# DataIntensive-HPC/abft-sparse-cg

Hardware: AMD Instinct MI355X
Metric: CG iterations/sec + SpMV effective HBM GB/s (% of roofline), 1/2/4/8 MI355X (higher is better)
Workload: dtype f64; 1 GPU; cg-csr -t hip -m none, synthetic laplace5:3162,3162; N=9998244, nnz=49978572, format=csr, mode=none, parallelism=1 GPU

## Files before the change

abft_sparse_cg_amd/capi.py:

```python
import ctypes as C
import os

_HERE = os.path.dirname(os.path.abspath(__file__))
LIB_PATH = os.environ.get("ABFT_HIP_LIB") or os.path.join(_HERE, "libabft_hip.so")
HEADER_PATH = os.path.join(os.path.dirname(_HERE), "include", "abft_hip.h")

OK = 0
MODES = ("none", "constraints", "sed", "sec7", "sec8", "secded")
MODE_ID = {m: i for i, m in enumerate(MODES)}
MODE_ID["sec"] = MODE_ID["sec7"]
FMT_CSR, FMT_COO = 0, 1
FLIP_ANY, FLIP_VALUE, FLIP_INDEX = 0, 1, 2
PART_ALL, PART_INTERIOR, PART_BOUNDARY = 0, 1, 2
K_SPMV, K_DOT, K_CALC_XR, K_CALC_P = 0, 1, 2, 3
EV_VEC_CORRECTED, EV_VEC_DOUBLE = 10, 11
FMT_VECTOR = 2
MAX_RHS = 8

u32p = C.POINTER(C.c_uint32)
f64p = C.POINTER(C.c_double)
i32p = C.POINTER(C.c_int)
vp = C.c_void_p
vpp = C.POINTER(C.c_void_p)

# ... 9 lines not shown

    def tup(self):
        return (self.kind, self.index, self.bit)


SIGNATURES = {
    "abft_hip_last_error": (C.c_char_p, []),
    "abft_hip_device_count": (C.c_int, [i32p]),
    "abft_hip_init": (C.c_int, [C.c_int, vpp]),
    "abft_hip_shutdown": (C.c_int, [vp]),
    "abft_hip_set_stream": (C.c_int, [vp, vp]),
    "abft_hip_get_stream": (vp, [vp]),
    "abft_hip_synchronize": (C.c_int, [vp]),
    "abft_hip_synchronize_timeout": (C.c_int, [vp, C.c_double]),
    "abft_hip_matrix_create_csr": (C.c_int, [vp, C.c_int, u32p, u32p, f64p, C.c_int, C.c_int, vpp]),
    "abft_hip_matrix_create_coo": (C.c_int, [vp, C.c_int, u32p, u32p, f64p, C.c_int, C.c_int, vpp]),
    "abft_hip_matrix_create_shard": (C.c_int, [vp, C.c_int, C.c_int, u32p, u32p, f64p, C.c_int, C.c_int,
                                               C.c_int, C.c_uint32, vpp]),
    "abft_hip_matrix_create_shard_indexed": (C.c_int, [vp, C.c_int, C.c_int, u32p, u32p, f64p, C.c_int, C.c_int,
                                                       C.c_int, u32p, vpp]),
    "abft_hip_matrix_destroy": (C.c_int, [vp]),
    "abft_hip_matrix_info": (C.c_int, [vp, i32p, i32p]),
    "abft_hip_matrix_compact_stats": (C.c_int, [vp, u32p, u32p, u32p]),
    "abft_hip_matrix_packed_stats": (C.c_int, [vp, u32p, u32p, u32p]),
    "abft_hip_matrix_read_element": (C.c_int, [vp, C.c_uint32, u32p]),
    "abft_hip_matrix_read_csr": (C.c_int, [vp, vp, vp, vp]),
    "abft_hip_matrix_read_coo": (C.c_int, [vp, vp]),
    "abft_hip_inject": (C.c_int, [vp, C.c_uint32, i32p, C.c_int]),
    "abft_hip_inject_rowptr": (C.c_int, [vp, C.c_uint32, C.c_uint32]),
    "abft_hip_vector_create": (C.c_int, [vp, C.c_int, vpp]),
    "abft_hip_vector_view": (C.c_int, [vp, C.c_int, C.c_int, vpp]),
    "abft_hip_vector_destroy": (C.c_int, [vp]),
    "abft_hip_vector_map": (C.c_int, [vp, C.POINTER(f64p)]),
    "abft_hip_vector_unmap": (C.c_int, [vp, f64p]),
    "abft_hip_vector_copy": (C.c_int, [vp, vp]),
    "abft_hip_vector_device_ptr": (vp, [vp]),
    "abft_hip_vector_length": (C.c_int, [vp]),
    "abft_hip_dot": (C.c_int, [vp, vp, vp, f64p]),
    "abft_hip_calc_xr": (C.c_int, [vp, vp, vp, vp, vp, C.c_double, f64p]),
    "abft_hip_calc_p": (C.c_int, [vp, vp, vp, C.c_double]),
    "abft_hip_spmv": (C.c_int, [vp, vp, vp, vp]),
    "abft_hip_matrix_create_csr_stream": (C.c_int, [vp, C.c_int, u32p, u32p, f64p, C.c_int, C.c_int, vpp]),
    "abft_hip_spmm": (C.c_int, [vp, vp, vp, vp, C.c_int]),
    "abft_hip_dot_block": (C.c_int, [vp, vp, vp, C.c_int, f64p]),
    "abft_hip_calc_xr_block": (C.c_int, [vp, vp, vp, vp, vp, C.c_int, f64p, C.c_uint32, f64p]),
    "abft_hip_calc_p_block": (C.c_int, [vp, vp, vp, C.c_int, f64p, C.c_uint32]),
    "abft_hip_vector_flip": (C.c_int, [vp, C.c_int, i32p, C.c_int]),
    "abft_hip_vector_encode": (C.c_int, [vp, vp]),
    "abft_hip_vector_scrub": (C.c_int, [vp, vp, i32p, i32p]),
    "abft_hip_spmv_vecc": (C.c_int, [vp, vp, vp, vp]),
    "abft_hip_dot_vecc": (C.c_int, [vp, vp, vp, f64p]),
    "abft_hip_calc_xr_vecc": (C.c_int, [vp, vp, vp, vp, vp, C.c_double, f64p]),
    "abft_hip_calc_p_vecc": (C.c_int, [vp, vp, vp, C.c_double]),
    "abft_hip_residual_gap": (C.c_int, [vp, vp, vp, vp, vp, vp, f64p]),
    "abft_hip_residual_restart": (C.c_int, [vp, vp, vp, vp, vp, vp, vp, f64p]),
    "abft_hip_residual_gap_block": (C.c_int, [vp, vp, vp, vp, vp, vp, C.c_int, C.c_uint32, f64p]),
    "abft_hip_residual_restart_block": (C.c_int, [vp, vp, vp, vp, vp, vp, vp, C.c_int, C.c_uint32, f64p]),
    "abft_hip_copy_block": (C.c_int, [vp, vp, vp, C.c_int, C.c_uint32]),
    "abft_hip_matrix_diag_inverse": (C.c_int, [vp, vp, vp, u32p]),
    "abft_hip_precond_start": (C.c_int, [vp, vp, vp, vp, f64p]),
    "abft_hip_calc_xr_precond": (C.c_int, [vp, vp, vp, vp, vp, vp, C.c_double, f64p]),
    "abft_hip_calc_p_precond": (C.c_int, [vp, vp, vp, vp, C.c_double]),
    "abft_hip_precond_start_block": (C.c_int, [vp, vp, vp, vp, C.c_int, C.c_uint32, f64p]),
    "abft_hip_calc_xr_precond_block": (C.c_int, [vp, vp, vp, vp, vp, vp, C.c_int, f64p, C.c_uint32, f64p]),
    "abft_hip_calc_p_precond_block": (C.c_int, [vp, vp, vp, vp, C.c_int, f64p, C.c_uint32]),
    "abft_hip_spmm_dot": (C.c_int, [vp, vp, vp, vp, C.c_int, f64p]),
    "abft_hip_calc_r_block": (C.c_int, [vp, vp, vp, C.c_int, f64p, C.c_uint32, f64p]),
    "abft_hip_calc_px_block": (C.c_int, [vp, vp, vp, vp, C.c_int, f64p, f64p, C.c_uint32]),
    "abft_hip_calc_r_precond_block": (C.c_int, [vp, vp, vp, vp, C.c_int, f64p, C.c_uint32, f64p]),
    "abft_hip_calc_px_precond_block": (C.c_int, [vp, vp, vp, vp, vp, C.c_int, f64p, f64p, C.c_uint32]),
    "abft_hip_dot_dev": (C.c_int, [vp, vp, vp, vp]),
    "abft_hip_calc_xr_dev": (C.c_int, [vp, vp, vp, vp, vp, C.c_double, vp]),
    "abft_hip_read_pair": (C.c_int, [vp, vp, f64p, f64p]),
    "abft_hip_spmv_dot_dev": (C.c_int, [vp, vp, vp, vp, C.c_int, vp]),
    "abft_hip_matrix_set_interior": (C.c_int, [vp, C.c_int, C.c_int]),
    "abft_hip_spmv_part": (C.c_int, [vp, vp, vp, vp, C.c_int]),
    "abft_hip_spmv_dot_part_dev": (C.c_int, [vp, vp, vp, vp, C.c_int, vp, C.c_int]),
    "abft_hip_calc_xr_ratio_dev": (C.c_int, [vp, vp, vp, vp, vp, vp, vp, vp]),
    "abft_hip_calc_p_ratio_dev": (C.c_int, [vp, vp, vp, vp, vp]),
    "abft_hip_set_sharers": (C.c_int, [vp, C.c_int]),
    "abft_hip_speculation_stats": (C.c_int, [vp, C.POINTER(C.c_long), C.POINTER(C.c_long)]),
    "abft_hip_cg_iteration_dev": (C.c_int, [vp, vp, vp, C.c_int, C.c_int, vp, vp, vp, vp, vp, vp, vp]),
    "abft_hip_tail_stats": (C.c_int, [vp, i32p, i32p, i32p, C.POINTER(C.c_long)]),
    "abft_hip_cg_iteration_until_dev": (C.c_int, [vp, vp, vp, C.c_int, C.c_int, vp, vp, vp, vp, vp, vp, vp, C.c_double]),
    "abft_hip_write_pair": (C.c_int, [vp, vp, C.c_double, C.c_double]),
    "abft_hip_peer_board_bytes": (C.c_size_t, []),
    "abft_hip_peer_board_attach": (C.c_int, [vp, vp, C.c_size_t, C.c_int, C.c_int, C.c_double]),
    "abft_hip_peer_board_detach": (C.c_int, [vp]),
    "abft_hip_allreduce_pair_peers": (C.c_int, [vp, vp]),
    "abft_hip_peer_board_failed": (C.c_int, [vp]),
    "abft_hip_peer_board_ipc_handle_bytes": (C.c_size_t, []),
    "abft_hip_peer_board_ipc_export": (C.c_int, [vp, vp]),
    "abft_hip_peer_board_ipc_attach": (C.c_int, [vp, vp, C.c_int, C.c_int, C.c_double]),
    "abft_hip_peer_board_device_alloc": (C.c_int, [vp, C.POINTER(vp)]),
    "abft_hip_peer_board_device_free": (C.c_int, [vp, vp]),
    "abft_hip_peer_board_attach_device": (C.c_int, [vp, C.POINTER(vp), C.c_int, C.c_int, C.c_double]),
    "abft_hip_peer_board_fuse": (C.c_int, [vp, C.c_int]),
    "abft_hip_peer_exchange_bytes": (C.c_size_t, [C.c_int, C.c_size_t]),
    "abft_hip_peer_exchange_attach": (C.c_int, [vp, vp, C.c_size_t, C.c_int, C.c_int, C.c_size_t, vp, C.c_int, vp,
                                                C.c_int, C.c_double]),
    "abft_hip_peer_exchange_detach": (C.c_int, [vp]),
    "abft_hip_peer_exchange": (C.c_int, [vp, vp]),
    "abft_hip_peer_exchange_begin": (C.c_int, [vp, vp, C.c_int]),
    "abft_hip_peer_exchange_finish": (C.c_int, [vp]),
    "abft_hip_peer_exchange_failed": (C.c_int, [vp]),
    "abft_hip_peer_exchange_ipc_export": (C.c_int, [vp, C.c_int, C.c_size_t, vp]),
    "abft_hip_peer_exchange_ipc_attach": (C.c_int, [vp, vp, C.c_int, C.c_int, C.c_size_t, vp, C.c_int, vp, C.c_int,
                                                    C.c_double]),
    "abft_hip_peer_exchange_device_alloc": (C.c_int, [vp, C.c_int, C.c_size_t, C.POINTER(vp)]),
    "abft_hip_peer_exchange_device_free": (C.c_int, [vp, vp]),
    "abft_hip_peer_exchange_attach_device": (C.c_int, [vp, C.POINTER(vp), C.c_int, C.c_int, C.c_size_t, vp, C.c_int, vp,
                                                       C.c_int, C.c_double]),
    "abft_hip_matrix_panels": (C.c_int, [vp, i32p, i32p]),
    "abft_hip_spmv_dot_range_dev": (C.c_int, [vp, vp, vp, vp, C.c_int, vp, C.c_int, C.c_int]),
    "abft_hip_graph_begin": (C.c_int, [vp]),
    "abft_hip_graph_end": (C.c_int, [vp, vpp]),
    "abft_hip_graph_launch": (C.c_int, [vp]),
    "abft_hip_graph_destroy": (C.c_int, [vp]),
    "abft_hip_drain_events": (C.c_int, [vp, C.POINTER(Event), C.c_int, i32p, i32p]),
    "abft_hip_event_capacity": (C.c_int, []),
    "abft_hip_pending_events": (C.c_int, [vp]),
    "abft_format_event": (C.c_int, [C.POINTER(Event), C.c_char_p, C.c_size_t]),
    "abft_event_is_fatal": (C.c_int, [C.c_uint32]),
    "abft_hip_profile_enable": (C.c_int, [vp, C.c_int]),
    "abft_hip_profile_stride": (C.c_int, [vp, C.c_int]),
    "abft_hip_profile_reset": (C.c_int, [vp]),
    "abft_hip_profile_read": (C.c_int, [vp, C.c_int, f64p, C.POINTER(C.c_long)]),
    "abft_hip_stream_probe": (C.c_int, [vp, C.c_size_t, C.c_int, f64p, f64p]),
}

_lib = None


def _share_torch_hip_runtime():
    if os.environ.get("ABFT_HIP_SYSTEM_RUNTIME") == "1":
        return
    import importlib.util
    try:
        spec = importlib.util.find_spec("torch")
    except Exception:
        spec = None
    if spec is None or not spec.origin:
        return
    rt = os.path.join(os.path.dirname(spec.origin), "lib", "libamdhip64.so")
    if os.path.exists(rt):
        C.CDLL(rt, mode=C.RTLD_GLOBAL)


def load():
    global _lib
    if _lib is None:
        if not os.path.exists(LIB_PATH):
            raise ImportError("%s not found: build it with `make -C %s` (hipcc --offload-arch=gfx950); "
                              "there is no CPU fallback" % (LIB_PATH, os.path.join(_HERE, "csrc")))
        _share_torch_hip_runtime()
        lib = C.CDLL(LIB_PATH)
        for name, (res, args) in SIGNATURES.items():
            fn = getattr(lib, name)
            fn.restype = res
            fn.argtypes = args
        _lib = lib
    return _lib


def check(rc):
    if rc != OK:
# ... 13 lines not shown
```

abft_sparse_cg_amd/context.py:

```python
import ctypes as C
import math
import sys

import numpy as np

from . import capi
from .capi import FMT_COO, FMT_CSR, MODE_ID, check


class FatalEvent(SystemExit):

    def __init__(self, events):
        super().__init__(1)
        self.events = events


class ResidualCheckFailed(RuntimeError):

    def __init__(self, message, checks):
        super().__init__(message)
        self.checks = checks


class Matrix:
# ... 351 lines not shown
        b = np.zeros(capi.MAX_RHS)
        b[:k] = beta
        check(self.L.abft_hip_calc_p_precond_block(self.h, p.h, r.h, dinv.h, k, b.ctypes.data_as(capi.f64p),
                                                   int(active)))

    def matrix_info(self, mat):
        lay, n = C.c_int(0), C.c_int(0)
        check(self.L.abft_hip_matrix_info(mat.h, C.byref(lay), C.byref(n)))
        return ("stream", "panels", "sweep", "slice")[lay.value], n.value

    def set_interior(self, mat, row_lo, row_hi):
        check(self.L.abft_hip_matrix_set_interior(mat.h, row_lo, row_hi))

    def inject_bitflip(self, mat, kind, num_flips):
        kind = self.BITFLIP.get(kind, kind)
        rand = self.rng or _libc_rand
        index = rand() % mat.nnz
        if mat.fmt == FMT_CSR:
            start, end = (0, 64) if kind == capi.FLIP_VALUE else (64, 96) if kind == capi.FLIP_INDEX else (0, 96)
        else:
            start, end = (64, 128) if kind == capi.FLIP_VALUE else (0, 64) if kind == capi.FLIP_INDEX else (0, 128)
        bits = []
        for _ in range(num_flips):
            bit = rand() % (end - start) + start
            sys.stdout.write("*** flipping bit %d at index %d ***\n" % (bit, index))
            bits.append(bit)
        self.inject_at(mat, index, bits)
        return index, bits

    def inject_at(self, mat, index, bits):
        b = np.ascontiguousarray(bits, dtype=np.int32)
        check(self.L.abft_hip_inject(mat.h, index, b.ctypes.data_as(capi.i32p), len(b)))

    def synchronize(self):
        check(self.L.abft_hip_synchronize(self.h))

    def drain_events(self):
        if self._evbuf is None:
            self._evcap = self.L.abft_hip_event_capacity()
            self._evbuf = (capi.Event * self._evcap)()
        n, fatal = C.c_int(0), C.c_int(0)
        check(self.L.abft_hip_drain_events(self.h, self._evbuf, self._evcap, C.byref(n), C.byref(fatal)))
        return [self._evbuf[i].tup() for i in range(n.value)], bool(fatal.value)

    def _drain_if_pending(self):
        if self.L.abft_hip_pending_events(self.h):
            self._drain()

    def _drain(self):
        events, fatal = self.drain_events()
        if not events:
            return
        self.event_log.extend(events)
        if self.on_event is not None:
            self.on_event(events, fatal)
            return
        for k, i, b in events:
            sys.stdout.write(capi.format_event(k, i, b, self.fmt))
        if fatal:
            sys.stdout.flush()
            raise FatalEvent(events)

    def profile(self, mask=0xF, stride=1):
        self.prof_mask = 0xF if mask is True else int(mask)
        check(self.L.abft_hip_profile_stride(self.h, stride))
        check(self.L.abft_hip_profile_enable(self.h, self.prof_mask))
        check(self.L.abft_hip_profile_reset(self.h))

    def profile_read(self, kernel):
        ms, n = C.c_double(), C.c_long()
        check(self.L.abft_hip_profile_read(self.h, kernel, C.byref(ms), C.byref(n)))
        return ms.value, n.value

    def stream_probe(self, nbytes=1 << 30, reps=10):
        c, r = C.c_double(), C.c_double()
        check(self.L.abft_hip_stream_probe(self.h, nbytes, reps, C.byref(c), C.byref(r)))
        return c.value, r.value

    def tail_stats(self):
        path, grid, want = C.c_int(0), C.c_int(0), C.c_int(0)
        counts = (C.c_long * 4)()
        check(self.L.abft_hip_tail_stats(self.h, C.byref(path), C.byref(grid), C.byref(want), counts))
        return path.value, grid.value, want.value, list(counts)

    def cg_iteration_until_dev(self, mat, vec, x, r, p, w, scalars, rr_at, pw_at, rr_new_at, threshold, vec_offset=0,
                               part=capi.PART_ALL):
        base = scalars.device_ptr
        check(self.L.abft_hip_cg_iteration_until_dev(self.h, mat.h, vec.h, vec_offset, part, x.h, r.h, p.h, w.h,
                                                     base + 8 * rr_at, base + 8 * pw_at, base + 8 * rr_new_at,
                                                     threshold))

    def graph_begin(self):
        check(self.L.abft_hip_graph_begin(self.h))

    def graph_end(self):
        g = C.c_void_p()
        check(self.L.abft_hip_graph_end(self.h, C.byref(g)))
        return g

    def graph_launch(self, graph):
        check(self.L.abft_hip_graph_launch(graph))

    def graph_destroy(self, graph):
        check(self.L.abft_hip_graph_destroy(graph))

    @property
    def stream(self):
        return self.L.abft_hip_get_stream(self.h)


_libc = None


def _libc_rand():
    global _libc
    if _libc is None:
        _libc = C.CDLL(None)
    return _libc.rand()


def vecc_strip(array):
    words = np.ascontiguousarray(array, dtype=np.float64).view(np.uint64) & np.uint64(0xFFFFFFFFFFFFFF80)
    return words.view(np.float64)


def fdiv(a, b):
    if b == 0.0:
        a = float(a)
        return float("nan") if a == 0.0 or a != a else float("inf") if (a > 0) == (str(float(b))[0] != "-") else float("-inf")
    return a / b


def threshold_ambiguous(rr, conv_threshold):
    return conv_threshold > 0.0 and abs(rr - conv_threshold) <= 1e-12 * abs(rr)


def note_threshold(rr, conv_threshold, state):
    import sys
    if not state.get("noted") and threshold_ambiguous(rr, conv_threshold):
        state["noted"] = True
        sys.stderr.write("note: threshold-ambiguous run: rr = %s is within 1e-12 (relative) of the convergence "
                         "threshold %.17g; the reference's serially summed rr may fall on the other side and run "
                         "one iteration more or fewer\n" % (float(rr).hex(), conv_threshold))


def _check_passes(gap2, tt2, bb, check_tol):
    return (gap2 <= check_tol * check_tol * bb) and math.isfinite(gap2) and math.isfinite(tt2)


def _ckpt_name(itr):
    return "the start" if itr < 0 else "iteration %d" % itr


def _check_args(check_every, check_tol, max_rollbacks):
    if check_every < 0 or int(check_every) != check_every:
        raise ValueError("check_every must be a whole number >= 0, not %r" % (check_every,))
    if not check_tol > 0 or not math.isfinite(check_tol):
        raise ValueError("check_tol must be a positive number, not %r" % (check_tol,))
    if max_rollbacks < 0:
        raise ValueError("max_rollbacks must be >= 0, not %r" % (max_rollbacks,))


def cg_solve(ctx, A, b, x, r, p, w, max_itrs=1000, conv_threshold=1e-3, on_iteration=None, check_every=0,
             check_tol=1e-7, max_rollbacks=3, x_ckpt=None, on_check=None, precond=None, vector_ecc=False):
    _check_args(check_every, check_tol, max_rollbacks)
    if vector_ecc:
# ... 300 lines not shown
```

abft_sparse_cg_amd/csrc/abft_hip.hip:

```cpp
#include <algorithm>
#include <array>
#include <chrono>
#include <cmath>
#include <cstdarg>
#include <cstdio>
#include <cstdlib>
#include <cstring>
#include <new>
#include <thread>
#include <map>
#include <mutex>
#include <vector>

#include "abft_internal.h"


static thread_local char g_err[512] = "";

static int set_err(int code, const char *fmt, ...) {
  va_list ap;
  va_start(ap, fmt);
  vsnprintf(g_err, sizeof(g_err), fmt, ap);
  va_end(ap);
  return code;
}

#define HIPCHK(call)                                                                   \
  do {                                                                                 \
    hipError_t e_ = (call);                                                            \
    if (e_ != hipSuccess)                                                              \
      return set_err(ABFT_ERR_HIP, "%s failed: %s (%s:%d)", #call, hipGetErrorString(e_), \
                     __FILE__, __LINE__);                                              \
  } while (0)

extern "C" const char *abft_hip_last_error(void) { return g_err; }


struct ProfSlot {
  std::vector<std::pair<hipEvent_t, hipEvent_t>> pending;
  double total_ms = 0.0;
  long launches = 0;
};

static constexpr uint32_t ABFT_HOST_SLOTS = 4;

struct abft_hip_ctx {
  int device = 0;
  int num_cus = 256;
  hipStream_t own_stream = nullptr, stream = nullptr;
  double *partials = nullptr;
  uint32_t *ticket = nullptr;
  unsigned long long *tail_sync = nullptr;
  bool capturing = false;
  bool tail_enabled = true;
  int tail_cap[3][3] = {{-1, -1, -1}, {-1, -1, -1}, {-1, -1, -1}};
  int sharers = 1;
  struct { int path = 0; uint32_t grid = 0, want = 0; long counts[4] = {0, 0, 0, 0}; } tail_stats;
  uint32_t seq = 0;
  bool spin_wait = true;
  HostSlot *host_slot = nullptr;
  HostSlot *host_slot_dev = nullptr;
  struct {
    bool enabled = false;
    bool learned = false;
    abft_hip_vector *x = nullptr, *r = nullptr, *p = nullptr, *w = nullptr;
    bool have_rr = false;
    int rr_at = 0;
    double rr_host = 0.0;
    int stage = 0;
    uint32_t seq_rr = 0;
    double rr_new_host = 0.0;
    double *shadow[2] = {nullptr, nullptr};
    int shadow_n = 0;
    double *scal = nullptr;
    long commits = 0, drops = 0;
  } spec;
  EventRing ring{};
  MovedList moved{};
  int *bits_dev = nullptr;
  bool fuse_enabled = true;
  struct {
    bool valid = false, have_value = false;
    bool vecc = false;
    const double *x = nullptr, *y = nullptr;
    int n = 0;
    uint32_t seq = 0;
    double value = 0.0;
  } fused;
  bool defer_enabled = true;
  struct {
    bool active = false, on_dev = false;
    double *x = nullptr;
    const double *p = nullptr;
    int n = 0;
    double alpha = 0.0;
  } defer;
  double *alpha_dev = nullptr;
  double *bpartials = nullptr;
  HostSlotK *bslot = nullptr, *bslot_dev = nullptr;
  HostSlotW *wslot = nullptr, *wslot_dev = nullptr;
  uint32_t bseq = 0;
  double *dotparts = nullptr;
  size_t dotparts_cap = 0;
  unsigned prof = 0;
  unsigned prof_stride = 1, prof_seen[ABFT_K_COUNT] = {};
  ProfSlot prof_k[ABFT_K_COUNT];
  std::vector<hipEvent_t> ev_pool;
  struct {
    bool attached = false;
    void *host = nullptr;
    PeerSlot *dev = nullptr;
    PeerSlot **table = nullptr;
    bool own_local = false;
    std::vector<void *> opened;
    unsigned long long *counter = nullptr;
    int rank = 0, size = 0;
    unsigned long long timeout_ticks = 0;
    bool fuse = false;
  } peers;
  struct {
    bool attached = false;
    void *host = nullptr;
    unsigned char *local = nullptr;
    unsigned char **table = nullptr;
    bool own_local = false;
    std::vector<void *> opened;
    PeerExchange *dev = nullptr;
    unsigned long long *counter = nullptr;
    int rank = 0;
    size_t extent = 0;
    hipStream_t side = nullptr;
    hipEvent_t fork = nullptr, join = nullptr;
    bool pending = false;
  } xchg;
};

struct abft_hip_matrix {
  abft_hip_ctx *ctx = nullptr;
  int fmt = 0, mode = 0;
  CsrDev csr{};
  CooDev coo{};
  double *fuse_partials = nullptr;
  bool use_panels = false;
  bool coo_pc = false;
  bool coo_lean = false;
  CsrPanels panels{};
  uint32_t panel_grid = 0;
  uint32_t panel_chunk = 0;
  bool use_sweep = false;
  SweepLayout sweep{};
  int sweep_rpt = 8;
  uint32_t sweep_grid = 0, sweep_width = 0;
  bool use_slice = false;
  SliceLayout slice{};
  uint32_t slice_grid = 0, slice_width = 0;
  std::vector<uint4> blk_host;
  uint32_t t_lo = 0, t_hi = 0;
  CsrCompact compact{};
  std::vector<uint32_t> cbase_host;
  CsrPacked packed{};
  std::vector<uint2> pdesc_host;
  std::vector<uint64_t> pal_host;
  std::map<std::array<uint64_t, ABFT_PAL_ENTRIES>, uint32_t> pal_index;
  size_t pal_cap = 0;
  std::vector<void *> allocs;
};

struct abft_hip_vector {
  abft_hip_ctx *ctx = nullptr;
  double *d = nullptr;
  int n = 0;
  bool owns = true;
  double *host = nullptr;
  abft_hip_vector *root = nullptr;
  bool exposed = false;
  int views = 0;
};

static constexpr uint32_t EVENT_CAP = 1u << 16;
static constexpr size_t VECC_SEEN_BYTES = ABFT_VECC_SEEN_SLOTS * sizeof(unsigned long long);
static_assert(sizeof(abft_event) % sizeof(unsigned long long) == 0, "the table behind the events is 8-byte aligned");
static constexpr uint32_t MOVED_CAP = 4096;

static int flush_deferred(abft_hip_ctx *ctx) {
  if (!ctx->defer.active) return ABFT_OK;
  ctx->defer.active = false;
  HIPCHK(launch_axpy(ctx->defer.x, ctx->defer.p, ctx->defer.alpha, ctx->defer.on_dev ? ctx->alpha_dev : nullptr,
                     ctx->defer.n, ctx->stream));
  return ABFT_OK;
}

static bool same_bits(double a, double b) { return memcmp(&a, &b, sizeof(a)) == 0; }

static void spec_drop(abft_hip_ctx *ctx) {
  auto &S = ctx->spec;
  if (S.stage) S.drops++;
  if (S.stage == 2) {
    S.rr_at = 1 - S.rr_at;
    S.rr_host = S.rr_new_host;
  }
  S.stage = 0;
}
static void spec_forget(abft_hip_ctx *ctx) {
  spec_drop(ctx);
  ctx->spec.learned = false;
  ctx->spec.have_rr = false;
  ctx->spec.x = ctx->spec.r = ctx->spec.p = ctx->spec.w = nullptr;
}

static int bind(abft_hip_ctx *ctx, bool keep_deferred = false, bool keep_spec = false) {
  if (!ctx) return set_err(ABFT_ERR_INVALID, "null context");
  HIPCHK(hipSetDevice(ctx->device));
  if (!keep_spec) spec_drop(ctx);
  if (!keep_deferred) return flush_deferred(ctx);
  return ABFT_OK;
}


struct KernelTimer {
  abft_hip_ctx *ctx;
  int id;
  hipEvent_t a = nullptr, b = nullptr;
  KernelTimer(abft_hip_ctx *c, int k) : ctx(c), id(k) {
    if (!(ctx->prof >> id & 1u)) return;
    if (ctx->prof_seen[id]++ % ctx->prof_stride) return;
    a = take();
    b = take();
    if (a && b) (void)hipEventRecord(a, ctx->stream);
  }
  ~KernelTimer() {
    if (!a || !b) return;
    (void)hipEventRecord(b, ctx->stream);
    ctx->prof_k[id].pending.emplace_back(a, b);
    if (ctx->prof_k[id].pending.size() >= 4096) fold(ctx, id);
  }
  hipEvent_t take() {
    if (!ctx->ev_pool.empty()) {
      hipEvent_t e = ctx->ev_pool.back();
      ctx->ev_pool.pop_back();
      return e;
    }
    hipEvent_t e = nullptr;
    if (hipEventCreate(&e) != hipSuccess) return nullptr;
    return e;
  }
  static void fold(abft_hip_ctx *ctx, int id) {
    ProfSlot &p = ctx->prof_k[id];
    for (auto &pr : p.pending) {
      float ms = 0.f;
      if (hipEventSynchronize(pr.second) == hipSuccess &&
          hipEventElapsedTime(&ms, pr.first, pr.second) == hipSuccess) {
        p.total_ms += ms;
        p.launches++;
      }
      ctx->ev_pool.push_back(pr.first);
      ctx->ev_pool.push_back(pr.second);
    }
    p.pending.clear();
  }
};


static bool debug_leak(char what);
static std::mutex g_stream_mutex;
static std::vector<std::pair<int, hipStream_t>> g_stream_pool;

static hipStream_t pooled_stream_take(int device) {
  {
    std::lock_guard<std::mutex> lock(g_stream_mutex);
    for (size_t i = 0; i < g_stream_pool.size(); i++)
      if (g_stream_pool[i].first == device) {
        hipStream_t s = g_stream_pool[i].second;
        g_stream_pool.erase(g_stream_pool.begin() + (long)i);
        return s;
      }
  }
  hipStream_t s = nullptr;
  if (hipStreamCreateWithFlags(&s, hipStreamNonBlocking) != hipSuccess) return nullptr;
  return s;
}

static void pooled_stream_give_back(int device, hipStream_t s) {
  if (!s) return;
  if (debug_leak('S')) {
    (void)hipStreamDestroy(s);
    return;
  }
  std::lock_guard<std::mutex> lock(g_stream_mutex);
  g_stream_pool.emplace_back(device, s);
}

static bool debug_leak(char what) {
  static const char *e = getenv("ABFT_HIP_DEBUG_LEAK");
  return e && strchr(e, what);
}


extern "C" int abft_hip_device_count(int *count) {
  if (!count) return set_err(ABFT_ERR_INVALID, "null count");
  int n = 0;
  hipError_t e = hipGetDeviceCount(&n);
  if (e != hipSuccess) {
    *count = 0;
    return set_err(ABFT_ERR_NODEVICE, "hipGetDeviceCount: %s", hipGetErrorString(e));
  }
  *count = n;
  return ABFT_OK;
}

static ReduceOut reduce_out(abft_hip_ctx *ctx, double *dev_out, bool to_host);

extern "C" int abft_hip_init(int device, abft_hip_ctx **out) {
  if (!out) return set_err(ABFT_ERR_INVALID, "null out");
  *out = nullptr;
  int n = 0;
  if (hipGetDeviceCount(&n) != hipSuccess || n <= 0)
    return set_err(ABFT_ERR_NODEVICE, "no HIP device visible (this engine has no CPU fallback)");
  if (device < 0 || device >= n) return set_err(ABFT_ERR_INVALID, "device %d out of range [0,%d)", device, n);
  HIPCHK(hipSetDevice(device));
  hipDeviceProp_t prop;
  HIPCHK(hipGetDeviceProperties(&prop, device));
  if (strncmp(prop.gcnArchName, "gfx950", 6) != 0)
    return set_err(ABFT_ERR_NODEVICE, "device %d is %s; this library carries gfx950 code only", device,
                   prop.gcnArchName);
  abft_hip_ctx *ctx = new (std::nothrow) abft_hip_ctx();
  if (!ctx) return set_err(ABFT_ERR_NOMEM, "context allocation failed");
  ctx->device = device;
  ctx->num_cus = prop.multiProcessorCount > 0 ? prop.multiProcessorCount : 256;
  ctx->own_stream = pooled_stream_take(device);
  if (!ctx->own_stream) return set_err(ABFT_ERR_HIP, "hipStreamCreateWithFlags failed");
  ctx->stream = ctx->own_stream;
  HIPCHK(hipMalloc((void **)&ctx->partials, ABFT_MAX_PARTIALS * sizeof(double)));
  HIPCHK(hipMalloc((void **)&ctx->ticket, ABFT_TICKET_WORDS * sizeof(uint32_t)));
  HIPCHK(hipMemset(ctx->ticket, 0, ABFT_TICKET_WORDS * sizeof(uint32_t)));
  HIPCHK(hipMalloc((void **)&ctx->tail_sync, 64 * sizeof(unsigned long long)));
  HIPCHK(hipMemset(ctx->tail_sync, 0, 64 * sizeof(unsigned long long)));
  if (const char *e = getenv("ABFT_HIP_TAIL")) ctx->tail_enabled = strcmp(e, "0") != 0;
  if (const char *e = getenv("ABFT_HIP_SYNC")) ctx->spin_wait = strcmp(e, "stream") != 0;
  if (const char *e = getenv("ABFT_HIP_FUSE_DOT")) ctx->fuse_enabled = strcmp(e, "0") != 0;
  if (const char *e = getenv("ABFT_HIP_FUSE_X")) ctx->defer_enabled = strcmp(e, "0") != 0;
  HIPCHK(hipMalloc((void **)&ctx->alpha_dev, sizeof(double)));
  HIPCHK(hipHostMalloc((void **)&ctx->host_slot, ABFT_HOST_SLOTS * sizeof(HostSlot), hipHostMallocMapped | hipHostMallocCoherent));
  memset(ctx->host_slot, 0, ABFT_HOST_SLOTS * sizeof(HostSlot));
  HIPCHK(hipMalloc((void **)&ctx->spec.scal, 8 * sizeof(double)));
  HIPCHK(hipMemset(ctx->spec.scal, 0, 8 * sizeof(double)));
  if (const char *e = getenv("ABFT_HIP_SPECULATE")) ctx->spec.enabled = strcmp(e, "0") != 0;
  HIPCHK(hipHostGetDevicePointer((void **)&ctx->host_slot_dev, ctx->host_slot, 0));
  HIPCHK(hipMalloc((void **)&ctx->ring.buf, EVENT_CAP * sizeof(abft_event) + VECC_SEEN_BYTES));
  HIPCHK(hipMalloc((void **)&ctx->ring.count, sizeof(uint32_t)));
  HIPCHK(hipMemset(ctx->ring.count, 0, sizeof(uint32_t)));
  HIPCHK(hipMemset(ctx->ring.buf + EVENT_CAP, 0, VECC_SEEN_BYTES));
  ctx->ring.cap = EVENT_CAP;
  HIPCHK(hipMalloc((void **)&ctx->moved.buf, 2 * (size_t)MOVED_CAP * sizeof(MovedEntry)));
  HIPCHK(hipMalloc((void **)&ctx->moved.count, sizeof(uint32_t)));
  HIPCHK(hipMemset(ctx->moved.count, 0, sizeof(uint32_t)));
  ctx->moved.cap = MOVED_CAP;
  HIPCHK(hipMalloc((void **)&ctx->bits_dev, 32 * sizeof(int)));
  {
    double *scratch = nullptr;
    HIPCHK(hipMalloc((void **)&scratch, 8 * sizeof(double)));
    HIPCHK(hipMemset(scratch, 0, 8 * sizeof(double)));
    ReduceOut o = reduce_out(ctx, scratch + 6, false);
    HIPCHK(launch_dot(scratch, scratch + 2, 2, o, ctx->stream));
    HIPCHK(launch_calc_xr(scratch, scratch + 2, scratch + 4, scratch + 4, 0.0, nullptr, nullptr, 2, o, ctx->stream));
    HIPCHK(launch_calc_p(scratch, scratch + 2, 0.0, nullptr, nullptr, 2, ctx->stream));
    HIPCHK(launch_copy(scratch, scratch + 2, 2, ctx->stream));
    HIPCHK(hipStreamSynchronize(ctx->stream));
    HIPCHK(hipFree(scratch));
  }
  *out = ctx;
  return ABFT_OK;
}

extern "C" int abft_hip_shutdown(abft_hip_ctx *ctx) {
  if (!ctx) return ABFT_OK;
  (void)hipSetDevice(ctx->device);
  (void)flush_deferred(ctx);
  (void)hipStreamSynchronize(ctx->stream);
  if (debug_leak('d')) (void)hipDeviceSynchronize();
  for (int k = 0; k < ABFT_K_COUNT; k++) KernelTimer::fold(ctx, k);
  for (hipEvent_t e : ctx->ev_pool) (void)hipEventDestroy(e);
  (void)hipFree(ctx->partials);
  (void)hipFree(ctx->alpha_dev);
  (void)hipFree(ctx->ticket);
  if (getenv("ABFT_HIP_TAIL_DEBUG") && ctx->tail_sync) {
    unsigned long long w[64] = {0};
    if (hipMemcpy(w, ctx->tail_sync, sizeof(w), hipMemcpyDeviceToHost) == hipSuccess && w[40])
      fprintf(stderr, "cg_tail phases of the last launch (us, workgroup 0): loads issued %.2f, p.w known %.2f, r stored + partial out %.2f, "
              "arrived %.2f, all arrived %.2f, r.r known %.2f, stores issued %.2f\n", 0.01 * (double)(w[41] - w[40]),
              0.01 * (double)(w[42] - w[40]), 0.01 * (double)(w[43] - w[40]), 0.01 * (double)(w[44] - w[40]),
              0.01 * (double)(w[45] - w[40]), 0.01 * (double)(w[46] - w[40]), 0.01 * (double)(w[47] - w[40]));
  }
  (void)hipFree(ctx->tail_sync);
  (void)hipFree(ctx->bpartials);
  (void)hipFree(ctx->dotparts);
  if (ctx->bslot) (void)hipHostFree(ctx->bslot);
  if (ctx->wslot) (void)hipHostFree(ctx->wslot);
  if (getenv("ABFT_HIP_VERBOSE") && (ctx->spec.commits || ctx->spec.drops))
    fprintf(stderr, "hip: speculated iterations: %ld taken over, %ld dropped\n", ctx->spec.commits, ctx->spec.drops);
  for (double *b : ctx->spec.shadow) (void)hipFree(b);
  (void)hipFree(ctx->spec.scal);
  if (!debug_leak('h')) (void)hipHostFree(ctx->host_slot);
  (void)hipFree(ctx->ring.buf);
  (void)hipFree(ctx->ring.count);
  (void)hipFree(ctx->moved.buf);
  (void)hipFree(ctx->moved.count);
  (void)hipFree(ctx->bits_dev);
  (void)abft_hip_peer_board_detach(ctx);
  (void)abft_hip_peer_exchange_detach(ctx);
  (void)hipStreamSynchronize(ctx->own_stream);
  pooled_stream_give_back(ctx->device, ctx->own_stream);
  delete ctx;
  return ABFT_OK;
}

extern "C" int abft_hip_set_stream(abft_hip_ctx *ctx, void *hip_stream) {
  if (int rc = bind(ctx)) return rc;
  HIPCHK(hipStreamSynchronize(ctx->stream));
  ctx->stream = hip_stream ? (hipStream_t)hip_stream : ctx->own_stream;
  return ABFT_OK;
}

extern "C" void *abft_hip_get_stream(abft_hip_ctx *ctx) { return ctx ? (void *)ctx->stream : nullptr; }

extern "C" int abft_hip_synchronize(abft_hip_ctx *ctx) {
  if (int rc = bind(ctx)) return rc;
  HIPCHK(hipStreamSynchronize(ctx->stream));
  return ABFT_OK;
}

extern "C" int abft_hip_synchronize_timeout(abft_hip_ctx *ctx, double seconds) {
  if (int rc = bind(ctx)) return rc;
  const auto t0 = std::chrono::steady_clock::now();
  for (;;) {
    const hipError_t q = hipStreamQuery(ctx->stream);
    if (q == hipSuccess) return ABFT_OK;
    if (q != hipErrorNotReady) return set_err(ABFT_ERR_HIP, "stream failed: %s", hipGetErrorString(q));
    if (std::chrono::duration<double>(std::chrono::steady_clock::now() - t0).count() > seconds)
      return set_err(ABFT_ERR_HIP, "timed out after %.0f s waiting for the stream", seconds);
    std::this_thread::sleep_for(std::chrono::microseconds(200));
  }
}


template <typename T>
static int dev_upload(abft_hip_matrix *m, T **dst, const T *src, size_t count, size_t alloc_count) {
  T *p = nullptr;
  if (alloc_count < count) alloc_count = count;
  if (alloc_count == 0) alloc_count = 1;
  if (hipMalloc((void **)&p, alloc_count * sizeof(T)) != hipSuccess)
    return set_err(ABFT_ERR_NOMEM, "hipMalloc of %zu bytes failed", alloc_count * sizeof(T));
  m->allocs.push_back(p);
  if (alloc_count > count)
    HIPCHK(hipMemsetAsync(p + count, 0, (alloc_count - count) * sizeof(T), m->ctx->stream));
  if (count) HIPCHK(hipMemcpyAsync(p, src, count * sizeof(T), hipMemcpyHostToDevice, m->ctx->stream));
  *dst = p;
  return ABFT_OK;
}

static void matrix_free(abft_hip_matrix *m) {
  if (!m) return;
  if (m->use_sweep && m->sweep.debug) {
    uint32_t d[16] = {0};
    if (hipMemcpy(d, m->sweep.debug, sizeof(d), hipMemcpyDeviceToHost) == hipSuccess) {
      fprintf(stderr, "sweep pacing: %u workgroup exits, %u waits, %u unsuccessful polls (lag %u, %u panels, grid %u)\n",
              d[2], d[1], d[0], m->sweep.lag, m->sweep.npanels, m->sweep_grid);
      unsigned long long t[6];
      memcpy(t, d + 4, sizeof(t));
      if (t[5])
        fprintf(stderr, "sweep phases (%% of workgroup time): counts+scan %.1f, pacing %.1f, stage (loads, ECC, gathers, "
                "LDS writes) %.1f, barrier %.1f, row sums %.1f, rest %.1f\n", 100.0 * t[0] / t[5], 100.0 * t[1] / t[5],
                100.0 * t[2] / t[5], 100.0 * t[3] / t[5], 100.0 * t[4] / t[5],
                100.0 * (t[5] - t[0] - t[1] - t[2] - t[3] - t[4]) / t[5]);
      if (t[5] && m->sweep.debug_wg) {
        const uint32_t ng = std::min<uint32_t>(m->sweep_grid, m->sweep.ngroups);
        std::vector<unsigned long long> w(4u * (size_t)ng);
        if (hipMemcpy(w.data(), m->sweep.debug_wg, w.size() * sizeof(w[0]), hipMemcpyDeviceToHost) == hipSuccess) {
          std::vector<double> busy, stage;
          double by_xcd[8] = {0}, n_xcd[8] = {0}, mx_xcd[8] = {0};
          for (uint32_t g = 0; g < ng; g++) {
            if (!w[4u * g]) continue;
            const double b = (double)(w[4u * g] - w[4u * g + 1]);
            busy.push_back(b);
// ... 1220 lines not shown
        return set_err(ABFT_ERR_HIP, "stream failed while waiting for a reduction: %s", hipGetErrorString(q));
    }
  }
  const uint32_t got = __atomic_load_n(slot_seq, __ATOMIC_ACQUIRE);
  if (got != seq)
    return set_err(ABFT_ERR_HIP, "reduction %u finished without publishing its result (slot holds %u)", seq, got);
  return ABFT_OK;
}

static int scalar_from_host_slot(abft_hip_ctx *ctx, uint32_t seq, double *result) {
  HostSlot *slot = ctx->host_slot + (seq % ABFT_HOST_SLOTS);
  if (int rc = wait_published(ctx, &slot->seq, seq)) return rc;
  *result = slot->value;
  return ABFT_OK;
}

static int check_same(const abft_hip_vector *a, const abft_hip_vector *b, const char *what) {
  if (!a || !b) return set_err(ABFT_ERR_INVALID, "%s: null vector", what);
  if (a->n != b->n) return set_err(ABFT_ERR_INVALID, "%s: lengths differ (%d vs %d)", what, a->n, b->n);
  return ABFT_OK;
}

extern "C" int abft_hip_dot(abft_hip_ctx *ctx, const abft_hip_vector *a, const abft_hip_vector *b, double *result) {
  if (int rc = bind(ctx, false, true)) return rc;
  if (int rc = check_same(a, b, "dot")) { spec_drop(ctx); return rc; }
  if (!result) { spec_drop(ctx); return set_err(ABFT_ERR_INVALID, "null result"); }
  if (ctx->fused.valid && !ctx->fused.vecc && a->n == ctx->fused.n &&
      ((a->d == ctx->fused.x && b->d == ctx->fused.y) || (a->d == ctx->fused.y && b->d == ctx->fused.x))) {
    if (!ctx->fused.have_value) {
      if (int rc = scalar_from_host_slot(ctx, ctx->fused.seq, &ctx->fused.value)) return rc;
      ctx->fused.have_value = true;
    }
    *result = ctx->fused.value;
    return ABFT_OK;
  }
  spec_drop(ctx);
  if (!ctx->fused.have_value) ctx->fused.valid = false;
  auto &S = ctx->spec;
  const int at = S.have_rr ? 1 - S.rr_at : 0;
  const ReduceOut o = reduce_out(ctx, S.scal + 2 * at, true);
  {
    KernelTimer t(ctx, ABFT_K_DOT);
    HIPCHK(launch_dot(a->d, b->d, a->n, o, ctx->stream));
  }
  if (int rc = scalar_from_host_slot(ctx, o.seq, result)) { S.have_rr = false; return rc; }
  S.have_rr = true; S.rr_at = at; S.rr_host = *result;
  return ABFT_OK;
}

extern "C" int abft_hip_dot_dev(abft_hip_ctx *ctx, const abft_hip_vector *a, const abft_hip_vector *b, double *dev_result) {
  if (int rc = bind(ctx)) return rc;
  if (int rc = check_same(a, b, "dot")) return rc;
  if (!dev_result) return set_err(ABFT_ERR_INVALID, "null result");
  KernelTimer t(ctx, ABFT_K_DOT);
  HIPCHK(launch_dot(a->d, b->d, a->n, reduce_out(ctx, dev_result, false), ctx->stream));
  return ABFT_OK;
}

static bool disjoint(const abft_hip_vector *a, const abft_hip_vector *b) {
  return a->d + a->n <= b->d || b->d + b->n <= a->d;
}

static int calc_xr_launch(abft_hip_ctx *ctx, abft_hip_vector *x, abft_hip_vector *r, const abft_hip_vector *p,
                          const abft_hip_vector *w, double alpha, const ReduceOut &o,
                          const double *num = nullptr, const double *den = nullptr) {
  if (int rc = check_same(x, r, "calc_xr")) return rc;
  if (int rc = check_same(x, p, "calc_xr")) return rc;
  if (int rc = check_same(x, w, "calc_xr")) return rc;
  ctx->fused.valid = false;
  const bool defer = ctx->defer_enabled && x->n > 0 && !(x->root ? x->root : x)->exposed && disjoint(x, r) &&
                     disjoint(x, p) && disjoint(x, w) && disjoint(r, p);
  KernelTimer t(ctx, ABFT_K_CALC_XR);
  if (defer) {
    HIPCHK(launch_calc_r(r->d, w->d, alpha, num, den, num ? ctx->alpha_dev : nullptr, x->n, o, ctx->stream, nullptr, x->d, p->d));
    ctx->defer.active = true;
    ctx->defer.on_dev = num != nullptr;
    ctx->defer.x = x->d; ctx->defer.p = p->d; ctx->defer.n = x->n; ctx->defer.alpha = alpha;
    return ABFT_OK;
  }
  HIPCHK(launch_calc_xr(x->d, r->d, p->d, w->d, alpha, num, den, x->n, o, ctx->stream));
  return ABFT_OK;
}

static int calc_p_launch(abft_hip_ctx *ctx, abft_hip_vector *p, const abft_hip_vector *r, double beta,
                         const double *num, const double *den) {
  if (int rc = check_same(p, r, "calc_p")) return rc;
  ctx->fused.valid = false;
  if (ctx->defer.active) {
    abft_hip_vector xv;
    xv.d = ctx->defer.x; xv.n = ctx->defer.n;
    if (ctx->defer.p == p->d && ctx->defer.n == p->n && disjoint(&xv, r)) {
      ctx->defer.active = false;
      KernelTimer t(ctx, ABFT_K_CALC_P);
      HIPCHK(launch_calc_px(p->d, r->d, ctx->defer.x, beta, num, den, ctx->defer.alpha,
                            ctx->defer.on_dev ? ctx->alpha_dev : nullptr, p->n, ctx->stream));
      return ABFT_OK;
    }
    if (int rc = flush_deferred(ctx)) return rc;
  }
  KernelTimer t(ctx, ABFT_K_CALC_P);
  HIPCHK(launch_calc_p(p->d, r->d, beta, num, den, p->n, ctx->stream));
  return ABFT_OK;
}

extern "C" int abft_hip_calc_xr(abft_hip_ctx *ctx, abft_hip_vector *x, abft_hip_vector *r, const abft_hip_vector *p,
                                const abft_hip_vector *w, double alpha, double *result) {
  if (int rc = bind(ctx, false, true)) return rc;
  if (!result) { spec_drop(ctx); return set_err(ABFT_ERR_INVALID, "null result"); }
  auto &S = ctx->spec;
  if (S.stage == 1) {
    bool take = x == S.x && r == S.r && p == S.p && w == S.w && ctx->fused.valid;
    if (take && !ctx->fused.have_value) {
      take = scalar_from_host_slot(ctx, ctx->fused.seq, &ctx->fused.value) == ABFT_OK;
      ctx->fused.have_value = take;
    }
    take = take && same_bits(alpha, S.rr_host / ctx->fused.value);
    if (take) {
      {
        double *rr = S.scal + 2 * S.rr_at, *rr_dev_new = S.scal + 2 * (1 - S.rr_at);
        KernelTimer t(ctx, ABFT_K_CALC_P);
        HIPCHK(launch_calc_px(p->d, S.shadow[0], x->d, 0.0, rr_dev_new, rr, 0.0, ctx->alpha_dev, x->n, ctx->stream, S.shadow[1],
                              nullptr));
      }
      double rr_new = 0.0;
      if (int rc = scalar_from_host_slot(ctx, S.seq_rr, &rr_new)) { spec_drop(ctx); return rc; }
      std::swap(r->d, S.shadow[0]);
      ctx->fused.valid = false;
      S.stage = 2;
      S.rr_new_host = rr_new;
      *result = rr_new;
      return ABFT_OK;
    }
    spec_drop(ctx);
  } else
    spec_drop(ctx);
  const int at = S.have_rr ? 1 - S.rr_at : 0;
  const ReduceOut o = reduce_out(ctx, S.scal + 2 * at, true);
  if (int rc = calc_xr_launch(ctx, x, r, p, w, alpha, o)) { S.have_rr = false; return rc; }
  if (int rc = scalar_from_host_slot(ctx, o.seq, result)) { S.have_rr = false; return rc; }
  S.have_rr = true; S.rr_at = at; S.rr_host = *result;
  S.x = x; S.r = r; S.p = const_cast<abft_hip_vector *>(p); S.w = const_cast<abft_hip_vector *>(w);
  S.learned = false;
  return ABFT_OK;
}

extern "C" int abft_hip_calc_xr_dev(abft_hip_ctx *ctx, abft_hip_vector *x, abft_hip_vector *r,
                                    const abft_hip_vector *p, const abft_hip_vector *w, double alpha,
                                    double *dev_result) {
  if (int rc = bind(ctx)) return rc;
  if (!dev_result) return set_err(ABFT_ERR_INVALID, "null result");
  return calc_xr_launch(ctx, x, r, p, w, alpha, reduce_out(ctx, dev_result, false));
}

extern "C" int abft_hip_calc_p(abft_hip_ctx *ctx, abft_hip_vector *p, const abft_hip_vector *r, double beta) {
  if (int rc = bind(ctx, true, true)) return rc;
  auto &S = ctx->spec;
  if (S.stage == 2) {
    const bool take = p == S.p && r == S.r && same_bits(beta, S.rr_new_host / S.rr_host) && !ctx->defer.active;
    if (take) {
      std::swap(p->d, S.shadow[1]);
      ctx->fused.valid = false;
      S.stage = 0;
      S.rr_at = 1 - S.rr_at;
      S.rr_host = S.rr_new_host;
      S.commits++;
      return ABFT_OK;
    }
    spec_drop(ctx);
  } else
    spec_drop(ctx);
  const bool completes = S.have_rr && !S.learned && S.p == p && S.r == r && S.x && S.w;
  if (int rc = calc_p_launch(ctx, p, r, beta, nullptr, nullptr)) return rc;
  S.learned = completes || (S.learned && S.p == p && S.r == r);
  return ABFT_OK;
}
// ... 456 lines not shown
  return ABFT_OK;
}

extern "C" int abft_hip_peer_exchange(abft_hip_ctx *ctx, abft_hip_vector *full) {
  return abft_hip_peer_exchange_begin(ctx, full, 0);
}

extern "C" int abft_hip_peer_exchange_failed(abft_hip_ctx *ctx) {
  if (!ctx || !ctx->xchg.attached) return 0;
  const size_t off = 2 * ABFT_PEER_MAX_RANKS * sizeof(unsigned long long);
  if (!ctx->xchg.host) {
    uint32_t f = 0;
    (void)hipSetDevice(ctx->device);
    if (hipMemcpy(&f, reinterpret_cast<const uint32_t *>(ctx->xchg.local + off) + ctx->xchg.rank, sizeof(f),
                  hipMemcpyDeviceToHost) != hipSuccess) {
      (void)hipGetLastError();
      return 1;
    }
    return f != 0;
  }
  const volatile uint32_t *fail = reinterpret_cast<const volatile uint32_t *>(static_cast<unsigned char *>(ctx->xchg.host) + off);
  return fail[ctx->xchg.rank] != 0;
}


extern "C" int abft_hip_calc_xr_ratio_dev(abft_hip_ctx *ctx, abft_hip_vector *x, abft_hip_vector *r,
                                          const abft_hip_vector *p, const abft_hip_vector *w,
                                          const double *dev_num, const double *dev_den, double *dev_result) {
  if (int rc = bind(ctx)) return rc;
  if (!dev_num || !dev_den || !dev_result) return set_err(ABFT_ERR_INVALID, "null device scalar");
  return calc_xr_launch(ctx, x, r, p, w, 0.0, reduce_out(ctx, dev_result, false), dev_num, dev_den);
}

extern "C" int abft_hip_calc_p_ratio_dev(abft_hip_ctx *ctx, abft_hip_vector *p, const abft_hip_vector *r,
                                         const double *dev_num, const double *dev_den) {
  if (int rc = bind(ctx, true)) return rc;
  if (!dev_num || !dev_den) {
    (void)flush_deferred(ctx);
    return set_err(ABFT_ERR_INVALID, "null device scalar");
  }
  return calc_p_launch(ctx, p, r, 0.0, dev_num, dev_den);
}

static bool spec_plain(const abft_hip_vector *v, int n) {
  return v && v->owns && v->root == v && !v->exposed && v->views == 0 && v->n == n && v->d;
}

static int spec_launch(abft_hip_ctx *ctx, const abft_hip_vector *vec, const abft_hip_vector *result) {
  auto &S = ctx->spec;
  if (!S.enabled || !S.learned || !S.have_rr || S.stage || ctx->defer.active || ctx->capturing) return ABFT_OK;
  if (vec != S.p || result != S.w) return ABFT_OK;
  const int n = vec->n;
  if (n <= 0 || !spec_plain(S.x, n) || !spec_plain(S.r, n) || !spec_plain(S.p, n) || !spec_plain(S.w, n)) return ABFT_OK;
  if (S.shadow_n != n) {
    for (double *&b : S.shadow) { (void)hipFree(b); b = nullptr; }
    S.shadow_n = 0;
    for (double *&b : S.shadow)
      if (hipMalloc((void **)&b, ((size_t)n + 2) * sizeof(double)) != hipSuccess) {
        (void)hipGetLastError();
        for (double *&c : S.shadow) { (void)hipFree(c); c = nullptr; }
        S.enabled = false;
        return ABFT_OK;
      }
    S.shadow_n = n;
  }
  double *rr = S.scal + 2 * S.rr_at, *rr_new = S.scal + 2 * (1 - S.rr_at), *pw = S.scal + 4;
  const ReduceOut o = reduce_out(ctx, rr_new, true);
  {
    KernelTimer t(ctx, ABFT_K_CALC_XR);
    HIPCHK(launch_calc_r(S.r->d, S.w->d, 0.0, rr, pw, ctx->alpha_dev, n, o, ctx->stream, S.shadow[0], S.x->d, S.p->d));
  }
  S.stage = 1;
  S.seq_rr = o.seq;
  return ABFT_OK;
}

struct HeldFold {
  bool held = false;
  FuseOut fuse{};
  uint32_t nparts = 0;
  FixArgs fix{};
};

static int spmv_common(abft_hip_ctx *ctx, abft_hip_matrix *mat, const abft_hip_vector *vec,
                       abft_hip_vector *result, int vec_offset, double *dev_pair, int part = ABFT_PART_ALL,
                       int c0 = 0, int c1 = -1, HeldFold *hold = nullptr, bool vecc = false) {
  if (int rc = bind(ctx)) return rc;
  if (!mat || !vec || !result) return set_err(ABFT_ERR_INVALID, "spmv: null argument");
  if (vecc) {
    spec_forget(ctx);
    const char *layout = mat->fmt != ABFT_FMT_CSR ? "COO" : mat->use_slice ? "slice" : mat->use_sweep ? "sweep"
                         : mat->use_panels ? "panel" : nullptr;
    if (layout)
      return set_err(ABFT_ERR_INVALID, "spmv_vecc: a matrix in the %s layout (protected vectors run on CSR matrices "
                     "in the streaming layout only)", layout);
    if (!disjoint(vec, result)) return set_err(ABFT_ERR_INVALID, "spmv_vecc: input and output overlap");
  }
  if (part < ABFT_PART_ALL || part > ABFT_PART_BOUNDARY) return set_err(ABFT_ERR_INVALID, "spmv: unknown part %d", part);
  const uint32_t n_out = mat->fmt == ABFT_FMT_CSR ? mat->csr.n_out : mat->coo.n_out;
  const uint32_t n_in = mat->fmt == ABFT_FMT_CSR ? mat->csr.n_in : mat->coo.n_in;
  if ((uint32_t)vec->n < n_in || (uint32_t)result->n < n_out)
    return set_err(ABFT_ERR_INVALID, "spmv: vectors (%d in, %d out) shorter than the matrix (%u in, %u out)",
                   vec->n, result->n, n_in, n_out);
  if (vec->d == result->d) return set_err(ABFT_ERR_INVALID, "spmv: input and output alias");
  if (dev_pair && (vec_offset < 0 || (uint64_t)vec_offset + n_out > (uint64_t)vec->n))
    return set_err(ABFT_ERR_INVALID, "spmv_dot: window [%d,%llu) outside the input vector of %d", vec_offset,
                   (unsigned long long)vec_offset + n_out, vec->n);
  ctx->fused.valid = false;
  FuseOut fuse{};
  const bool to_host = !dev_pair && ctx->fuse_enabled && n_in == n_out && (uint32_t)vec->n == n_in &&
                       (uint32_t)result->n == n_out;
  const bool want_fuse = mat->fuse_partials && (dev_pair || to_host);
  if (dev_pair && !want_fuse) return set_err(ABFT_ERR_INVALID, "spmv_dot: matrix has no rows");
  const uint32_t n_int = mat->t_hi - mat->t_lo;
  if (part == ABFT_PART_INTERIOR && n_int == 0) return ABFT_OK;
  const uint32_t npan = mat->use_sweep ? mat->sweep.npanels : mat->use_slice ? mat->slice.npanels : 1u;
  const bool whole = c1 < 0;
  if (whole) { c0 = 0; c1 = (int)npan; }
  if (c0 < 0 || c0 >= c1 || (uint32_t)c1 > npan) return set_err(ABFT_ERR_INVALID, "spmv: panels [%d,%d) outside [0,%u)", c0, c1, npan);
  if (!whole && part != ABFT_PART_ALL) return set_err(ABFT_ERR_INVALID, "spmv: a panel range with a row part");
  if (!whole && mat->mode == ABFT_MODE_CONSTRAINTS && c1 - c0 < (int)npan)
    return set_err(ABFT_ERR_INVALID, "spmv: a panel range in constraints mode");
  const bool last_range = (uint32_t)c1 == npan;
  const bool do_fuse = want_fuse && last_range;
  TileSpan span{0u, mat->csr.nblk, 0u, mat->csr.nblk};
  if (part == ABFT_PART_INTERIOR) span = TileSpan{mat->t_lo, n_int, 0u, n_int};
  else if (part == ABFT_PART_BOUNDARY && n_int) span = TileSpan{0u, mat->t_lo, n_int, mat->csr.nblk - n_int};
  if (do_fuse) {
    fuse.partials = mat->fuse_partials;
    fuse.ev_count = ctx->ring.count;
    fuse.seq = dev_pair ? 0 : ++ctx->seq;
    fuse.host = dev_pair ? nullptr : ctx->host_slot_dev + (fuse.seq % ABFT_HOST_SLOTS);
    fuse.dev_out = dev_pair ? dev_pair : ctx->spec.scal + 4;
    fuse.x_off = dev_pair ? (uint32_t)vec_offset : 0u;
    if (dev_pair && ctx->peers.fuse) fuse.peers = peer_args(ctx);
  }
  uint32_t nparts = mat->fmt == ABFT_FMT_CSR ? mat->csr.nblk : mat->coo.nblk;
  FixArgs fix{};
  {
    KernelTimer t(ctx, ABFT_K_SPMV);
    if (mat->use_slice) {
      nparts = mat->slice_grid;
      HIPCHK(launch_spmv_slice(mat->mode, mat->csr, mat->slice, vec->d, result->d, ctx->ring, do_fuse ? &fuse : nullptr,
                               mat->slice_grid, (uint32_t)c0, (uint32_t)c1, ctx->stream));
    } else if (mat->use_sweep) {
      nparts = mat->sweep_grid;
      HIPCHK(launch_spmv_sweep(mat->mode, mat->sweep_rpt, mat->csr, mat->sweep, vec->d, result->d, ctx->ring,
                               do_fuse ? &fuse : nullptr, mat->sweep_grid, (uint32_t)c0, (uint32_t)c1, ctx->stream));
    } else if (mat->fmt == ABFT_FMT_CSR && mat->use_panels) {
      nparts = mat->panel_grid;
      HIPCHK(launch_spmv_csr_panels(mat->mode, mat->csr, mat->panels, vec->d, result->d, ctx->ring,
                                    do_fuse ? &fuse : nullptr, mat->panel_grid, mat->panel_chunk, ctx->stream));
    } else if (mat->fmt == ABFT_FMT_COO && mat->use_panels) {
      nparts = mat->panel_grid;
      if (mat->coo_pc)
        HIPCHK(launch_spmv_coo_pc(mat->mode, mat->coo, mat->panels, vec->d, result->d, ctx->ring,
                                  do_fuse ? &fuse : nullptr, mat->panel_grid, mat->panel_chunk, ctx->stream));
      else if (mat->coo_lean)
        HIPCHK(launch_spmv_coo_lean(mat->mode, mat->coo, mat->panels, vec->d, result->d, ctx->ring,
                                    do_fuse ? &fuse : nullptr, mat->panel_grid, mat->panel_chunk, ctx->stream));
      else
        HIPCHK(launch_spmv_coo_panels(mat->mode, mat->coo, mat->panels, vec->d, result->d, ctx->ring,
                                      do_fuse ? &fuse : nullptr, mat->panel_grid, mat->panel_chunk, ctx->stream));
    } else if (mat->fmt == ABFT_FMT_CSR)
      HIPCHK(launch_spmv_csr(mat->mode, mat->csr, mat->compact, mat->packed, span, vec->d, result->d, ctx->ring,
                             do_fuse ? &fuse : nullptr, ctx->stream, vecc));
    else
      HIPCHK(launch_spmv_coo(mat->mode, mat->coo, vec->d, result->d, ctx->ring, do_fuse ? &fuse : nullptr, ctx->stream));
    if (mat->fmt == ABFT_FMT_COO) {
      fix = make_fix_args(mat->mode, mat->coo, mat->use_panels ? &mat->panels : nullptr, vec->d, result->d,
                          do_fuse ? &fuse : nullptr);
      if (!do_fuse) HIPCHK(launch_coo_fixup(fix, ctx->stream));
    }
  }
  if (part == ABFT_PART_INTERIOR || !last_range) return ABFT_OK;
  if (do_fuse && hold) {
    hold->held = true;
    hold->fuse = fuse;
    hold->nparts = nparts;
    hold->fix = fix;
    return ABFT_OK;
  }
  if (do_fuse) {
    KernelTimer t(ctx, ABFT_K_DOT);
    ReduceOut big{};
    big.partials = ctx->partials; big.ticket = ctx->ticket; big.dev_out = fuse.dev_out; big.host = fuse.host;
    big.ev_count = fuse.ev_count; big.seq = fuse.seq; big.peers = fuse.peers;
    HIPCHK(launch_fuse_finalize(fuse, nparts, big, fix.on ? &fix : nullptr, ctx->stream));
  }
  if (to_host && do_fuse) {
    ctx->fused.valid = true;
    ctx->fused.have_value = false;
    ctx->fused.vecc = vecc;
    ctx->fused.x = vec->d;
    ctx->fused.y = result->d;
    ctx->fused.n = vec->n;
    ctx->fused.seq = fuse.seq;
    if (whole && part == ABFT_PART_ALL && !vecc) (void)spec_launch(ctx, vec, result);
  }
  return ABFT_OK;
}

extern "C" int abft_hip_spmv(abft_hip_ctx *ctx, abft_hip_matrix *mat, const abft_hip_vector *vec,
                             abft_hip_vector *result) {
  return spmv_common(ctx, mat, vec, result, 0, nullptr);
}

extern "C" int abft_hip_spmv_dot_dev(abft_hip_ctx *ctx, abft_hip_matrix *mat, const abft_hip_vector *vec,
                                     abft_hip_vector *result, int vec_offset, double *dev_result) {
  if (!dev_result) return set_err(ABFT_ERR_INVALID, "null result");
  return spmv_common(ctx, mat, vec, result, vec_offset, dev_result);
}


static int check_block(const char *what, int k, int N, std::initializer_list<const abft_hip_vector *> vs) {
  if (k < 1 || k > ABFT_MAX_RHS) return set_err(ABFT_ERR_INVALID, "%s: k = %d outside [1, %d]", what, k, ABFT_MAX_RHS);
  if (N < 0 || (int64_t)N * k >= ((int64_t)1 << 31))
    return set_err(ABFT_ERR_INVALID, "%s: %d rows x %d columns does not fit a block vector", what, N, k);
  for (const abft_hip_vector *v : vs) {
    if (!v) return set_err(ABFT_ERR_INVALID, "%s: null vector", what);
    if ((int64_t)v->n != (int64_t)N * k)
      return set_err(ABFT_ERR_INVALID, "%s: a vector of length %d is not a block of %d rows x %d columns", what, v->n,
                     N, k);
    if (k % 2 == 0 && ((uintptr_t)v->d & 15u))
      return set_err(ABFT_ERR_INVALID, "%s: a block vector with an even k must start 16-byte aligned (a view at an "
                     "odd offset does not)", what);
  }
  return ABFT_OK;
}

static int bind_block(abft_hip_ctx *ctx) {
  if (int rc = bind(ctx)) return rc;
  ctx->fused.valid = false;
  spec_forget(ctx);
  return ABFT_OK;
}

static int block_slot(abft_hip_ctx *ctx) {
  if (ctx->bslot) return ABFT_OK;
  HIPCHK(hipMalloc((void **)&ctx->bpartials, (size_t)2 * ABFT_MAX_RHS * ABFT_MAX_PARTIALS * sizeof(double)));
  HIPCHK(hipHostMalloc((void **)&ctx->wslot, sizeof(HostSlotW), hipHostMallocMapped | hipHostMallocCoherent));
  memset(ctx->wslot, 0, sizeof(HostSlotW));
  HIPCHK(hipHostGetDevicePointer((void **)&ctx->wslot_dev, ctx->wslot, 0));
  HIPCHK(hipHostMalloc((void **)&ctx->bslot, sizeof(HostSlotK), hipHostMallocMapped | hipHostMallocCoherent));
  memset(ctx->bslot, 0, sizeof(HostSlotK));
  HIPCHK(hipHostGetDevicePointer((void **)&ctx->bslot_dev, ctx->bslot, 0));
  return ABFT_OK;
}

static ReduceOutK reduce_out_k(abft_hip_ctx *ctx) {
// ... 361 lines not shown
        d[i] = 1.0;
        nbad++;
      }
    }
    HIPCHK(hipMemcpyAsync(dinv->d, d.data(), (size_t)N * sizeof(double), hipMemcpyHostToDevice, s));
    HIPCHK(hipStreamSynchronize(s));
    *bad = nbad;
    return ABFT_OK;
  }
  uint32_t *count = reinterpret_cast<uint32_t *>(ctx->bits_dev);
  HIPCHK(hipMemsetAsync(count, 0, sizeof(uint32_t), s));
  HIPCHK(mat->fmt == ABFT_FMT_CSR ? launch_diag_csr(mat->csr, colmask, dinv->d, count, s)
                                  : launch_diag_coo(mat->coo, colmask, dinv->d, count, s));
  HIPCHK(hipMemcpyAsync(bad, count, sizeof(uint32_t), hipMemcpyDeviceToHost, s));
  HIPCHK(hipStreamSynchronize(s));
  return ABFT_OK;
}

static int bind_precond(abft_hip_ctx *ctx, bool keep_deferred = false) {
  if (int rc = bind(ctx, keep_deferred)) return rc;
  ctx->fused.valid = false;
  spec_forget(ctx);
  return ABFT_OK;
}

static int check_precond(const char *what, std::initializer_list<const abft_hip_vector *> reads,
                         std::initializer_list<const abft_hip_vector *> writes, const abft_hip_vector *dinv) {
  if (!dinv) return set_err(ABFT_ERR_INVALID, "%s: null vector", what);
  for (const abft_hip_vector *v : reads)
    if (int rc = check_same(v, dinv, what)) return rc;
  for (const abft_hip_vector *v : writes) {
    if (int rc = check_same(v, dinv, what)) return rc;
    if (dinv->n && !disjoint(v, dinv))
      return set_err(ABFT_ERR_INVALID, "%s: dinv overlaps a vector the call writes", what);
  }
  return ABFT_OK;
}

static int pair_from_block_slot(abft_hip_ctx *ctx, uint32_t seq, double out[2]) {
  return results_from_block_slot(ctx, seq, 2, out);
}

extern "C" int abft_hip_precond_start(abft_hip_ctx *ctx, const abft_hip_vector *r, const abft_hip_vector *dinv,
                                      abft_hip_vector *p, double out[2]) {
  if (!out) return set_err(ABFT_ERR_INVALID, "precond_start: null result");
  if (int rc = check_precond("precond_start", {r}, {p}, dinv)) return rc;
  if (r->n && !disjoint(r, p)) return set_err(ABFT_ERR_INVALID, "precond_start: r and p overlap");
  if (int rc = bind_precond(ctx)) return rc;
  if (int rc = block_slot(ctx)) return rc;
  const ReduceOutK o = reduce_out_k(ctx);
  {
    KernelTimer t(ctx, ABFT_K_DOT);
    HIPCHK(launch_precond_start(r->d, dinv->d, p->d, r->n, o, ctx->stream));
  }
  return pair_from_block_slot(ctx, o.seq, out);
}

extern "C" int abft_hip_calc_xr_precond(abft_hip_ctx *ctx, abft_hip_vector *x, abft_hip_vector *r,
                                        const abft_hip_vector *p, const abft_hip_vector *w,
                                        const abft_hip_vector *dinv, double alpha, double out[2]) {
  if (!out) return set_err(ABFT_ERR_INVALID, "calc_xr_precond: null result");
  if (int rc = check_precond("calc_xr_precond", {p, w}, {x, r}, dinv)) return rc;
  if (int rc = bind_precond(ctx)) return rc;
  if (int rc = block_slot(ctx)) return rc;
  const bool defer = ctx->defer_enabled && x->n > 0 && !(x->root ? x->root : x)->exposed && disjoint(x, r) &&
                     disjoint(x, p) && disjoint(x, w) && disjoint(r, p);
  const ReduceOutK o = reduce_out_k(ctx);
  {
    KernelTimer t(ctx, ABFT_K_CALC_XR);
    HIPCHK(launch_calc_xr_precond(defer ? nullptr : x->d, r->d, p->d, w->d, dinv->d, alpha, x->n, o, ctx->stream));
  }
  if (defer) {
    ctx->defer.active = true;
    ctx->defer.on_dev = false;
    ctx->defer.x = x->d; ctx->defer.p = p->d; ctx->defer.n = x->n; ctx->defer.alpha = alpha;
  }
  return pair_from_block_slot(ctx, o.seq, out);
}

extern "C" int abft_hip_calc_p_precond(abft_hip_ctx *ctx, abft_hip_vector *p, const abft_hip_vector *r,
                                       const abft_hip_vector *dinv, double beta) {
  if (int rc = check_precond("calc_p_precond", {r}, {p}, dinv)) return rc;
  if (int rc = bind_precond(ctx, true)) return rc;
  if (ctx->defer.active) {
    abft_hip_vector xv;
    xv.d = ctx->defer.x; xv.n = ctx->defer.n;
    if (ctx->defer.p == p->d && ctx->defer.n == p->n && !ctx->defer.on_dev && disjoint(&xv, r) && disjoint(&xv, dinv)) {
      ctx->defer.active = false;
      KernelTimer t(ctx, ABFT_K_CALC_P);
      HIPCHK(launch_calc_p_precond(p->d, r->d, dinv->d, ctx->defer.x, beta, ctx->defer.alpha, p->n, ctx->stream));
      return ABFT_OK;
    }
    if (int rc = flush_deferred(ctx)) return rc;
  }
  KernelTimer t(ctx, ABFT_K_CALC_P);
  HIPCHK(launch_calc_p_precond(p->d, r->d, dinv->d, nullptr, beta, 0.0, p->n, ctx->stream));
  return ABFT_OK;
}

static int check_precond_block(const char *what, int k, std::initializer_list<const abft_hip_vector *> reads,
                               std::initializer_list<const abft_hip_vector *> writes, const abft_hip_vector *dinv) {
  if (!dinv) return set_err(ABFT_ERR_INVALID, "%s: null vector", what);
  if (k < 1 || k > ABFT_MAX_RHS) return set_err(ABFT_ERR_INVALID, "%s: k = %d outside [1, %d]", what, k, ABFT_MAX_RHS);
  const int N = dinv->n;
  if (int rc = check_block(what, k, N, reads)) return rc;
  if (int rc = check_block(what, k, N, writes)) return rc;
  for (const abft_hip_vector *v : writes)
    if (N && !disjoint(v, dinv)) return set_err(ABFT_ERR_INVALID, "%s: dinv overlaps a vector the call writes", what);
  return ABFT_OK;
}

static ReduceOutW reduce_out_w(abft_hip_ctx *ctx) {
  ReduceOutW o{};
  o.partials = ctx->bpartials;
  o.ticket = ctx->ticket;
  o.host = ctx->wslot_dev;
  o.ev_count = ctx->ring.count;
  o.seq = ++ctx->bseq;
  return o;
}

static int results_from_wide_slot(abft_hip_ctx *ctx, uint32_t seq, int count, double *out) {
  if (int rc = wait_published(ctx, &ctx->wslot->seq, seq)) return rc;
  for (int j = 0; j < count; j++) out[j] = ctx->wslot->value[j];
  return ABFT_OK;
}

extern "C" int abft_hip_precond_start_block(abft_hip_ctx *ctx, const abft_hip_vector *R, const abft_hip_vector *dinv,
                                            abft_hip_vector *P, int k, uint32_t mask, double *out) {
  if (!out) return set_err(ABFT_ERR_INVALID, "precond_start_block: null result");
  if (int rc = check_precond_block("precond_start_block", k, {R}, {P}, dinv)) return rc;
  if (R->n && !disjoint(R, P)) return set_err(ABFT_ERR_INVALID, "precond_start_block: R and P overlap");
  if (int rc = bind_precond(ctx)) return rc;
  if (int rc = block_slot(ctx)) return rc;
  const ReduceOutW o = reduce_out_w(ctx);
  {
    KernelTimer t(ctx, ABFT_K_DOT);
    HIPCHK(launch_precond_start_block(R->d, dinv->d, P->d, dinv->n, k, mask, o, ctx->stream));
  }
  return results_from_wide_slot(ctx, o.seq, 2 * k, out);
}

extern "C" int abft_hip_calc_xr_precond_block(abft_hip_ctx *ctx, abft_hip_vector *X, abft_hip_vector *R,
                                              const abft_hip_vector *P, const abft_hip_vector *W,
                                              const abft_hip_vector *dinv, int k, const double *alpha, uint32_t active,
                                              double *out) {
  if (!alpha || !out) return set_err(ABFT_ERR_INVALID, "calc_xr_precond_block: null argument");
  if (int rc = check_precond_block("calc_xr_precond_block", k, {P, W}, {X, R}, dinv)) return rc;
  if (X->n && (!disjoint(X, R) || !disjoint(X, P) || !disjoint(X, W) || !disjoint(R, P) || !disjoint(R, W)))
    return set_err(ABFT_ERR_INVALID, "calc_xr_precond_block: x and r must not overlap each other or p, w");
  if (int rc = bind_precond(ctx)) return rc;
  if (int rc = block_slot(ctx)) return rc;
  BlockScalars a{};
  for (int j = 0; j < k; j++) a.v[j] = alpha[j];
  const ReduceOutW o = reduce_out_w(ctx);
  {
    KernelTimer t(ctx, ABFT_K_CALC_XR);
    HIPCHK(launch_calc_xr_precond_block(X->d, R->d, P->d, W->d, dinv->d, dinv->n, k, a, active, o, ctx->stream));
  }
  return results_from_wide_slot(ctx, o.seq, 2 * k, out);
}

extern "C" int abft_hip_calc_p_precond_block(abft_hip_ctx *ctx, abft_hip_vector *P, const abft_hip_vector *R,
                                             const abft_hip_vector *dinv, int k, const double *beta, uint32_t active) {
  if (!beta) return set_err(ABFT_ERR_INVALID, "calc_p_precond_block: null argument");
  if (int rc = check_precond_block("calc_p_precond_block", k, {R}, {P}, dinv)) return rc;
// ... 229 lines not shown
      ReduceOut big{};
      big.partials = ctx->partials; big.ticket = ctx->ticket; big.dev_out = hold.fuse.dev_out; big.host = hold.fuse.host;
      big.ev_count = hold.fuse.ev_count; big.seq = hold.fuse.seq; big.peers = hold.fuse.peers;
      HIPCHK(launch_fuse_finalize(hold.fuse, hold.nparts, big, hold.fix.on ? &hold.fix : nullptr, ctx->stream));
    }
    if (int rc = calc_xr_launch(ctx, x, r, p, w, 0.0, o, dev_rr, dev_pw)) return rc;
    return calc_p_launch(ctx, p, r, 0.0, dev_rr_new, dev_rr);
  }
  ctx->fused.valid = false;
  TailArgs a{};
  a.f = hold.fuse;
  a.nparts = hold.nparts;
  if (hold.nparts > 8192u) {
    uint32_t nb = (hold.nparts + 2047u) / 2048u;
    if (nb > 64u) nb = 64u;
    a.fold_nb = nb;
    a.fold_chunk = (hold.nparts + nb - 1u) / nb;
  }
  a.fx = hold.fix;
  a.o = o;
  a.rr = dev_rr;
  a.x = x->d; a.r = r->d; a.p = p->d; a.w = w->d;
  a.n = n;
  a.nbv = nbv;
  a.sync = ctx->tail_sync;
  a.timeout_ticks = 500000000ull;
  KernelTimer t(ctx, ABFT_K_CALC_XR);
  HIPCHK(launch_cg_tail(a, vec2, fast, q, grid, ctx->stream));
  return ABFT_OK;
}

extern "C" int abft_hip_cg_iteration_until_dev(abft_hip_ctx *ctx, abft_hip_matrix *mat, const abft_hip_vector *vec,
                                               int vec_offset, int part, abft_hip_vector *x, abft_hip_vector *r,
                                               abft_hip_vector *p, abft_hip_vector *w, const double *dev_rr,
                                               double *dev_pw, double *dev_rr_new, double threshold) {
  const char *what = "cg_iteration_until";
  if (int rc = bind(ctx)) return rc;
  if (!mat || !vec || !x || !r || !p || !w) return set_err(ABFT_ERR_INVALID, "%s: null argument", what);
  if (!dev_rr || !dev_pw || !dev_rr_new) return set_err(ABFT_ERR_INVALID, "%s: null device scalar", what);
  if (part != ABFT_PART_ALL && part != ABFT_PART_BOUNDARY)
    return set_err(ABFT_ERR_INVALID, "%s: part %d (the interior part goes through abft_hip_spmv_dot_part_dev)", what, part);
  if (ctx->peers.attached)
    return set_err(ABFT_ERR_INVALID, "%s: a peer board is attached; the guarded iteration runs on one rank", what);
  auto apart = [](const double *a, const double *b) { return a + 2 <= b || b + 2 <= a; };
  if (!apart(dev_rr, dev_pw) || !apart(dev_rr, dev_rr_new) || !apart(dev_pw, dev_rr_new))
    return set_err(ABFT_ERR_INVALID, "%s: the scalar pairs overlap", what);
  if (int rc = check_same(x, r, what)) return rc;
  if (int rc = check_same(x, p, what)) return rc;
  if (int rc = check_same(x, w, what)) return rc;
  const int n = x->n;
  const uint32_t n_out = mat->fmt == ABFT_FMT_CSR ? mat->csr.n_out : mat->coo.n_out;
  if ((uint32_t)n != n_out)
    return set_err(ABFT_ERR_INVALID, "%s: vectors of %d entries for a matrix of %u rows", what, n, n_out);
  if (vec_offset < 0 || (uint64_t)vec_offset + n_out > (uint64_t)vec->n)
    return set_err(ABFT_ERR_INVALID, "%s: window [%d,%llu) outside the input vector of %d", what, vec_offset,
                   (unsigned long long)vec_offset + n_out, vec->n);
  if (n > 0) {
    if (!disjoint(x, r) || !disjoint(x, p) || !disjoint(x, w) || !disjoint(r, p) || !disjoint(r, w) || !disjoint(p, w))
      return set_err(ABFT_ERR_INVALID, "%s: x, r, p and w overlap", what);
    if (!disjoint(vec, x) || !disjoint(vec, r) || !disjoint(vec, w))
      return set_err(ABFT_ERR_INVALID, "%s: the input vector overlaps x, r or w", what);
    if (!disjoint(vec, p) && p->d != vec->d + vec_offset)
      return set_err(ABFT_ERR_INVALID, "%s: p overlaps the input vector without being its window", what);
  }
  HeldFold hold;
  if (int rc = spmv_common(ctx, mat, vec, w, vec_offset, dev_pw, part, 0, -1, &hold)) return rc;
  if (hold.held) {
    KernelTimer t(ctx, ABFT_K_DOT);
    ReduceOut big{};
    big.partials = ctx->partials; big.ticket = ctx->ticket; big.dev_out = hold.fuse.dev_out; big.host = hold.fuse.host;
    big.ev_count = hold.fuse.ev_count; big.seq = hold.fuse.seq; big.peers = hold.fuse.peers;
    HIPCHK(launch_fuse_finalize(hold.fuse, hold.nparts, big, hold.fix.on ? &hold.fix : nullptr, ctx->stream));
  }
  const ReduceOut o = reduce_out(ctx, dev_rr_new, false);
  {
    KernelTimer t(ctx, ABFT_K_CALC_XR);
    HIPCHK(launch_calc_r_until(r->d, w->d, dev_rr, dev_pw, threshold, ctx->alpha_dev, n, o, ctx->stream, x->d, p->d));
  }
  KernelTimer t(ctx, ABFT_K_CALC_P);
  HIPCHK(launch_calc_px_until(p->d, r->d, x->d, dev_rr, dev_rr_new, threshold, ctx->alpha_dev, n, ctx->stream));
  return ABFT_OK;
}


struct abft_hip_graph {
  abft_hip_ctx *ctx = nullptr;
  hipGraph_t graph = nullptr;
  hipGraphExec_t exec = nullptr;
};

extern "C" int abft_hip_graph_begin(abft_hip_ctx *ctx) {
  if (int rc = bind(ctx)) return rc;
  if (ctx->prof) return set_err(ABFT_ERR_INVALID, "graph capture with kernel brackets enabled (abft_hip_profile_enable)");
  HIPCHK(hipStreamBeginCapture(ctx->stream, hipStreamCaptureModeThreadLocal));
  ctx->capturing = true;
  return ABFT_OK;
}

extern "C" int abft_hip_graph_end(abft_hip_ctx *ctx, abft_hip_graph **out) {
  if (!ctx || !out) return set_err(ABFT_ERR_INVALID, "null argument");
  *out = nullptr;
  ctx->capturing = false;
  if (ctx->defer.active) {
    hipGraph_t g = nullptr;
    (void)hipStreamEndCapture(ctx->stream, &g);
    if (g) (void)hipGraphDestroy(g);
    ctx->defer.active = false;
    return set_err(ABFT_ERR_INVALID, "captured sequence ends with a deferred x update pending (calc_xr without its calc_p)");
  }
  hipGraph_t g = nullptr;
  HIPCHK(hipStreamEndCapture(ctx->stream, &g));
  abft_hip_graph *h = new (std::nothrow) abft_hip_graph();
  if (!h) { (void)hipGraphDestroy(g); return set_err(ABFT_ERR_NOMEM, "graph handle"); }
  h->ctx = ctx; h->graph = g;
  hipError_t e = hipGraphInstantiate(&h->exec, g, nullptr, nullptr, 0);
  if (e != hipSuccess) {
    (void)hipGraphDestroy(g);
    delete h;
    return set_err(ABFT_ERR_HIP, "hipGraphInstantiate: %s", hipGetErrorString(e));
  }
  *out = h;
  return ABFT_OK;
}

extern "C" int abft_hip_graph_launch(abft_hip_graph *g) {
  if (!g) return set_err(ABFT_ERR_INVALID, "null graph");
  if (int rc = bind(g->ctx)) return rc;
  g->ctx->fused.valid = false;
  HIPCHK(hipGraphLaunch(g->exec, g->ctx->stream));
  return ABFT_OK;
}

extern "C" int abft_hip_graph_destroy(abft_hip_graph *g) {
  if (!g) return ABFT_OK;
  (void)hipSetDevice(g->ctx->device);
  (void)hipStreamSynchronize(g->ctx->stream);
  if (g->exec) (void)hipGraphExecDestroy(g->exec);
  if (g->graph) (void)hipGraphDestroy(g->graph);
  delete g;
  return ABFT_OK;
}


extern "C" int abft_event_is_fatal(uint32_t kind) {
  return kind == ABFT_EV_SED_DETECTED || kind == ABFT_EV_DOUBLE_BIT || kind == ABFT_EV_VEC_DOUBLE ||
         (kind >= ABFT_EV_ROW_SIZE && kind <= ABFT_EV_MOVED_OVERFLOW);
}

extern "C" int abft_format_event(const abft_event *ev, char *buf, size_t cap) {
  if (!ev || !buf) return -1;
  const bool coo = ev->fmt == ABFT_FMT_COO;
  const int i = (int)ev->index;
  switch (ev->kind) {
    case ABFT_EV_SED_DETECTED: return snprintf(buf, cap, "[ECC] error detected at index %d\n", i);
    case ABFT_EV_CORRECTED_BIT: return snprintf(buf, cap, "[ECC] corrected bit %u at index %d\n", ev->bit, i);
    case ABFT_EV_CORRECTED_PARITY: return snprintf(buf, cap, "[ECC] corrected overall parity bit at index %d\n", i);
    case ABFT_EV_DOUBLE_BIT: return snprintf(buf, cap, "[ECC] double-bit error detected\n");
    case ABFT_EV_ROW_SIZE:
      return snprintf(buf, cap, coo ? "row size constraint violated for index %d\n"
                                    : "row size constraint violated for row %d\n", i);
    case ABFT_EV_ROW_ORDER:
      return snprintf(buf, cap, coo ? "row index order violated at index %d\n"
                                    : "row order constraint violated for row%d\n", i);
    case ABFT_EV_COL_SIZE:
      return snprintf(buf, cap, coo ? "column size constraint violated for index %d\n"
                                    : "column size constraint violated at index %d\n", i);
    case ABFT_EV_COL_ORDER:
      return snprintf(buf, cap, coo ? "column index order violated at index %d\n"
                                    : "column order constraint violated at index %d\n", i);
    case ABFT_EV_MOVED_OVERFLOW:
      return snprintf(buf, cap, "hip: more than %d COO elements carry a silently corrupted column\n", i);
    case ABFT_EV_VEC_CORRECTED:
      return snprintf(buf, cap, "[ECC] corrected bit %u of vector operand %u at index %d\n", ev->bit & 0xffu,
                      (ev->bit >> 8) & 0xffu, i);
    case ABFT_EV_VEC_DOUBLE:
      return snprintf(buf, cap, "[ECC] double-bit error detected in vector operand %u at index %d\n",
// ... 144 lines not shown
```

abft_sparse_cg_amd/csrc/abft_internal.h:

```cpp
#pragma once
#include <hip/hip_runtime.h>
#include <stdint.h>

#include "../../include/abft_hip.h"

struct EventRing {
  abft_event *buf;
  uint32_t *count;
  uint32_t cap;
};

#define ABFT_VECC_SEEN_SLOTS 4096u
#define ABFT_VECC_SEEN_PROBES 8u

struct CsrDev {
  uint32_t *cols;
  double *vals;
  const uint32_t *rowptr;
  const uint4 *blk;
  uint32_t nblk, n_out, n_in, nnz, index_base;
  const uint32_t *orig_index;
  const uint32_t *pos_of_orig;
  const uint32_t *gidx;
};
// ... 24 lines not shown
struct SweepLayout {
  const uint32_t *wbase;
  const uint8_t *counts;
  uint32_t ngroups, npanels;
  uint32_t *pace;
  uint32_t lag;
  uint32_t *debug;
  unsigned long long *debug_wg;
};

struct SliceLayout {
  const uint32_t *sub;
  const uint16_t *rid;
  uint32_t nslices, npanels, rows_log2;
  uint32_t *pace;
  uint32_t lag;
};

#ifndef ABFT_CFG_SLICE_K
#define ABFT_CFG_SLICE_K 2
#endif
#ifndef ABFT_CFG_SLICE_WAVES
#define ABFT_CFG_SLICE_WAVES 8
#endif

#ifndef ABFT_CFG_PANEL_RPT
#define ABFT_CFG_PANEL_RPT 8
#endif
constexpr int ABFT_PANEL_ROWS_PER_THREAD = ABFT_CFG_PANEL_RPT;
constexpr int ABFT_PANEL_ROWS = 256 * ABFT_PANEL_ROWS_PER_THREAD;

struct MovedEntry {
  uint32_t orig;
  uint32_t col;
  double prod;
};
struct MovedList {
  MovedEntry *buf;
  uint32_t *count;
  uint32_t cap;
};

struct CooDev {
  uint4 *elems;
  const uint32_t *grp_ptr;
  const uint4 *blk;
  const uint32_t *orig_index;
  const uint32_t *pos_of_orig;
  const uint2 *as_created;
  uint32_t nblk, n_out, n_in, nnz, index_base;
  MovedList moved;
  const uint32_t *gidx;
};

#define ABFT_COLMASK_HOST 0x00FFFFFFu

#ifndef ABFT_CFG_CSR_EPT
#define ABFT_CFG_CSR_EPT 4
#endif
#ifndef ABFT_CFG_PACKED_PAL
#define ABFT_CFG_PACKED_PAL 0
#endif
#ifndef ABFT_CFG_COO_EPT
#define ABFT_CFG_COO_EPT 4
#endif
#ifndef ABFT_CFG_PANEL_EPT
#define ABFT_CFG_PANEL_EPT 8
#endif
#ifndef ABFT_CFG_SWEEP_EPT
#define ABFT_CFG_SWEEP_EPT 8
#endif
#ifndef ABFT_CFG_COO_PANEL_EPT
#define ABFT_CFG_COO_PANEL_EPT 4
#endif
#ifndef ABFT_CFG_DEAD_NT
#define ABFT_CFG_DEAD_NT 0
#endif
#ifndef ABFT_CFG_SWEEP_COUNTS_NT
#define ABFT_CFG_SWEEP_COUNTS_NT 0
#endif
#ifndef ABFT_CFG_PX_OUT_NT
#define ABFT_CFG_PX_OUT_NT 0
#endif
#ifndef ABFT_CFG_X_NT
#define ABFT_CFG_X_NT 0
#endif
#ifndef ABFT_CFG_COO_LEAN_WAVES
#define ABFT_CFG_COO_LEAN_WAVES 8
#endif
#ifndef ABFT_CFG_COO_PANEL_XPF_AHEAD
#define ABFT_CFG_COO_PANEL_XPF_AHEAD 1
#endif
#ifndef ABFT_CFG_COO_PANEL_PREFETCH
#define ABFT_CFG_COO_PANEL_PREFETCH 0
#endif
#ifndef ABFT_CFG_COO_SCHED_BARRIER
#define ABFT_CFG_COO_SCHED_BARRIER 1
#endif
#ifndef ABFT_CFG_COO_PANEL_SHORT_SUMS
#define ABFT_CFG_COO_PANEL_SHORT_SUMS 1
#endif
#ifndef ABFT_CFG_SWEEP_SHORT_SUMS
#define ABFT_CFG_SWEEP_SHORT_SUMS 1
#endif
#ifndef ABFT_CFG_SWEEP_PREFETCH
#define ABFT_CFG_SWEEP_PREFETCH 0
#endif
#ifndef ABFT_CFG_SCHED_BARRIER
#define ABFT_CFG_SCHED_BARRIER 1
#endif
#ifndef ABFT_CFG_UNIFORM_ROWS
#define ABFT_CFG_UNIFORM_ROWS 1
#endif
#ifndef ABFT_CFG_NT
#define ABFT_CFG_NT 1
#endif
#ifndef ABFT_CFG_XCD
#define ABFT_CFG_XCD 1
#endif
#ifndef ABFT_CFG_XCD_CHUNK
#define ABFT_CFG_XCD_CHUNK 32
#endif

constexpr int ABFT_BLOCK = 256;
constexpr int ABFT_CSR_EPT = ABFT_CFG_CSR_EPT;
constexpr int ABFT_CSR_TILE = ABFT_BLOCK * ABFT_CSR_EPT;
constexpr int ABFT_COO_EPT = ABFT_CFG_COO_EPT;
constexpr int ABFT_COO_TILE = ABFT_BLOCK * ABFT_COO_EPT;
#ifndef ABFT_CFG_MAX_PARTIALS
#define ABFT_CFG_MAX_PARTIALS 2048
#endif
constexpr int ABFT_MAX_PARTIALS = ABFT_CFG_MAX_PARTIALS;
constexpr int ABFT_TICKET_GROUP = 32;
constexpr int ABFT_TICKET_WORDS = 1 + ABFT_MAX_PARTIALS / ABFT_TICKET_GROUP;

hipError_t launch_encode_csr(int mode, uint32_t *cols, double *vals, uint32_t nnz, hipStream_t s);
hipError_t launch_encode_coo(int mode, uint4 *elems, uint32_t nnz, hipStream_t s);
hipError_t launch_inject_csr(double *vals, uint32_t *cols, const uint32_t *pos_of_orig, uint32_t index,
                             const int *bits_dev, int nbits, hipStream_t s);
hipError_t launch_inject_coo(uint4 *elems, const uint32_t *pos_of_orig, uint32_t index,
                             const int *bits_dev, int nbits, hipStream_t s);

struct HostSlot {
  double value;
  uint32_t evcount;
  uint32_t seq;
};

#define ABFT_PEER_MAX_RANKS 64
struct PeerSlot {
  unsigned long long v0, v1, seq, pad;
};
#define ABFT_PEER_BOARD_BYTES (2 * ABFT_PEER_MAX_RANKS * sizeof(PeerSlot) + ABFT_PEER_MAX_RANKS * sizeof(uint32_t))
struct PeerArgs {
  PeerSlot *const *boards;
  PeerSlot *board;
  unsigned long long *counter;
  uint32_t *fail;
  int rank, size;
  unsigned long long timeout_ticks;
};

struct ReduceOut {
  double *partials;
  uint32_t *ticket;
  double *dev_out;
  HostSlot *host;
  const uint32_t *ev_count;
  uint32_t seq;
  PeerArgs peers;
};

struct FuseOut {
  double *partials;
  HostSlot *host;
  double *dev_out;
  const uint32_t *ev_count;
  uint32_t seq;
  uint32_t x_off;
  PeerArgs peers;
};

struct TileSpan {
  uint32_t first, cut, skip, count;
};

hipError_t launch_spmv_sweep(int mode, int rpt, const CsrDev &A, const SweepLayout &L, const double *x, double *y,
                             EventRing ev, const FuseOut *fuse, uint32_t grid, uint32_t c0, uint32_t c1, hipStream_t s);
int spmv_sweep_blocks_per_cu(int mode, int rpt);
hipError_t launch_spmv_slice(int mode, const CsrDev &A, const SliceLayout &L, const double *x, double *y, EventRing ev,
                             const FuseOut *fuse, uint32_t grid, uint32_t c0, uint32_t c1, hipStream_t s);
int spmv_slice_blocks_per_cu(int mode, uint32_t rows_log2);

hipError_t launch_spmv_csr_panels(int mode, const CsrDev &A, const CsrPanels &P, const double *x, double *y,
                                  EventRing ev, const FuseOut *fuse, uint32_t grid, uint32_t chunk,
                                  hipStream_t s);
int spmv_csr_panels_blocks_per_cu(int mode, bool fuse);
hipError_t launch_spmv_coo_panels(int mode, const CooDev &A, const CsrPanels &P, const double *x, double *y,
                                  EventRing ev, const FuseOut *fuse, uint32_t grid, uint32_t chunk,
                                  hipStream_t s);
struct FixArgs;
hipError_t launch_fuse_finalize(const FuseOut &f, uint32_t nblk, const ReduceOut &big, const FixArgs *fix, hipStream_t s);
hipError_t launch_spmv_csr(int mode, const CsrDev &A, const CsrCompact &cc, const CsrPacked &cp, const TileSpan &span,
                           const double *x, double *y, EventRing ev, const FuseOut *fuse, hipStream_t s,
                           bool vecc = false);
hipError_t launch_spmv_coo(int mode, const CooDev &A, const double *x, double *y, EventRing ev,
                           const FuseOut *fuse, hipStream_t s);
struct FixLayout {
  int kind;
  CsrPanels P;
};
struct FixArgs {
  CooDev A;
  FixLayout F;
  const double *x;
  double *y;
  double *partial0;
  uint32_t x_off;
  int ecc;
  int on;
};
FixArgs make_fix_args(int mode, const CooDev &A, const CsrPanels *P, const double *x, double *y, const FuseOut *fuse);
hipError_t launch_coo_fixup(const FixArgs &fx, hipStream_t s);

struct TailArgs {
  FuseOut f;
  uint32_t nparts;
  uint32_t fold_nb, fold_chunk;
  FixArgs fx;
  ReduceOut o;
  const double *rr;
  double *x, *r, *p;
  const double *w;
  int n;
  uint32_t nbv;
  unsigned long long *sync;
  unsigned long long timeout_ticks;
};
int spmv_coo_panels_blocks_per_cu(int mode);
int spmv_coo_pc_blocks_per_cu(int mode);
int spmv_coo_lean_blocks_per_cu(int mode);
hipError_t launch_spmv_coo_lean(int mode, const CooDev &A, const CsrPanels &P, const double *x, double *y, EventRing ev,
                                const FuseOut *fuse, uint32_t grid, uint32_t chunk, hipStream_t s);
hipError_t launch_spmv_coo_pc(int mode, const CooDev &A, const CsrPanels &P, const double *x, double *y, EventRing ev,
                              const FuseOut *fuse, uint32_t grid, uint32_t chunk, hipStream_t s);
int cg_tail_blocks_per_cu(bool vec2, bool fast, int q);
hipError_t launch_cg_tail(const TailArgs &a, bool vec2, bool fast, int q, uint32_t grid, hipStream_t s);

int reduce_blocks(int n);
hipError_t launch_dot(const double *a, const double *b, int n, const ReduceOut &out, hipStream_t s);
hipError_t launch_calc_xr(double *x, double *r, const double *p, const double *w, double alpha,
                          const double *num, const double *den, int n, const ReduceOut &out, hipStream_t s);
hipError_t launch_calc_p(double *p, const double *r, double beta, const double *num, const double *den, int n,
                         hipStream_t s);
hipError_t launch_calc_r(double *r, const double *w, double alpha, const double *num, const double *den,
                         double *alpha_out, int n, const ReduceOut &out, hipStream_t s, double *r_out = nullptr,
                         const double *x = nullptr, const double *p = nullptr);
hipError_t launch_calc_px(double *p, const double *r, double *x, double beta, const double *num, const double *den,
                          double alpha, const double *alpha_ptr, int n, hipStream_t s, double *p_out = nullptr,
                          double *x_out = nullptr);
hipError_t launch_axpy(double *x, const double *p, double alpha, const double *alpha_ptr, int n, hipStream_t s);
hipError_t launch_calc_r_until(double *r, const double *w, const double *rr, const double *pw, double threshold,
                               double *alpha_out, int n, const ReduceOut &out, hipStream_t s, const double *x,
                               const double *p);
hipError_t launch_calc_px_until(double *p, const double *r, double *x, const double *rr, const double *rr_new,
                                double threshold, const double *alpha_ptr, int n, hipStream_t s);

#define ABFT_MAX_RHS 8
struct HostSlotK {
  double value[ABFT_MAX_RHS];
  uint32_t evcount;
  uint32_t seq;
};
struct ReduceOutK {
  double *partials;
  uint32_t *ticket;
  HostSlotK *host;
  const uint32_t *ev_count;
  uint32_t seq;
};
struct BlockScalars {
  double v[ABFT_MAX_RHS];
};
hipError_t launch_spmm_csr(int mode, int k, const CsrDev &A, const double *x, double *y, EventRing ev, hipStream_t s);
hipError_t launch_dot_block(const double *a, const double *b, int n, int k, const ReduceOutK &out, hipStream_t s);
hipError_t launch_calc_xr_block(double *x, double *r, const double *p, const double *w, int n, int k,
                                const BlockScalars &alpha, uint32_t active, const ReduceOutK &out, hipStream_t s);
hipError_t launch_calc_p_block(double *p, const double *r, int n, int k, const BlockScalars &beta, uint32_t active,
                               hipStream_t s);
hipError_t launch_spmm_dot_csr(int mode, int k, const CsrDev &A, const double *x, double *y, EventRing ev,
                               double *dotp, hipStream_t s);
hipError_t launch_spmm_fold(const double *parts, uint32_t nblk, int k, const ReduceOutK &out, hipStream_t s);
hipError_t launch_calc_r_block(double *r, const double *w, int n, int k, const BlockScalars &alpha, uint32_t active,
                               const ReduceOutK &out, hipStream_t s);
hipError_t launch_calc_px_block(double *x, double *p, const double *r, const double *dinv, int n, int k,
                                const BlockScalars &alpha, const BlockScalars &beta, uint32_t active, hipStream_t s);
struct HostSlotW {
  double value[2 * ABFT_MAX_RHS];
  uint32_t evcount;
  uint32_t seq;
};
struct ReduceOutW {
  double *partials;
  uint32_t *ticket;
  HostSlotW *host;
  const uint32_t *ev_count;
  uint32_t seq;
};
hipError_t launch_flip_vector(double *v, unsigned long long mask, hipStream_t s);
hipError_t launch_vector_encode(double *v, int n, hipStream_t s);
hipError_t launch_vector_scrub(double *v, int n, uint32_t *counts, EventRing ev, hipStream_t s);
hipError_t launch_dot_vecc(const double *a, const double *b, int n, const ReduceOut &out, EventRing ev, hipStream_t s);
hipError_t launch_calc_xr_vecc(double *x, double *r, const double *p, const double *w, double alpha, int n,
                               const ReduceOut &out, EventRing ev, hipStream_t s);
hipError_t launch_calc_p_vecc(double *p, const double *r, double beta, int n, EventRing ev, hipStream_t s);
hipError_t launch_residual_gap(const double *b, const double *y, const double *r, int n, const ReduceOutK &out,
                               hipStream_t s);
hipError_t launch_residual_restart(const double *b, const double *y, double *r, double *p, int n, const ReduceOut &out,
                                   hipStream_t s);
hipError_t launch_residual_gap_block(const double *b, const double *y, const double *r, int n, int k, uint32_t active,
                                     const ReduceOutW &out, hipStream_t s);
hipError_t launch_residual_restart_block(const double *b, const double *y, double *r, double *p, int n, int k,
                                         uint32_t mask, const ReduceOutK &out, hipStream_t s);
hipError_t launch_copy_block(double *dst, const double *src, int n, int k, uint32_t mask, hipStream_t s);
hipError_t launch_precond_start(const double *r, const double *dinv, double *p, int n, const ReduceOutK &out,
                                hipStream_t s);
hipError_t launch_calc_xr_precond(double *x, double *r, const double *p, const double *w, const double *dinv,
                                  double alpha, int n, const ReduceOutK &out, hipStream_t s);
hipError_t launch_calc_p_precond(double *p, const double *r, const double *dinv, double *x, double beta, double alpha,
                                 int n, hipStream_t s);
hipError_t launch_precond_start_block(const double *r, const double *dinv, double *p, int n, int k, uint32_t mask,
                                      const ReduceOutW &out, hipStream_t s);
hipError_t launch_calc_xr_precond_block(double *x, double *r, const double *p, const double *w, const double *dinv,
                                        int n, int k, const BlockScalars &alpha, uint32_t active, const ReduceOutW &out,
                                        hipStream_t s);
hipError_t launch_calc_p_precond_block(double *p, const double *r, const double *dinv, int n, int k,
                                       const BlockScalars &beta, uint32_t active, hipStream_t s);
// ... 30 lines not shown
```

abft_sparse_cg_amd/csrc/kernels.hip:

```cpp
#include <type_traits>

#include "abft_internal.h"
#include "ecc_device.h"

typedef double f64x2 __attribute__((ext_vector_type(2)));
typedef uint32_t u32x2 __attribute__((ext_vector_type(2)));
typedef uint32_t u32x4 __attribute__((ext_vector_type(4)));

#if ABFT_CFG_NT
#define STREAM_LOAD(p) __builtin_nontemporal_load(p)
#else
#define STREAM_LOAD(p) (*(p))
#endif

#ifndef ABFT_CFG_GATHER
#define ABFT_CFG_GATHER 0
#endif
__device__ __forceinline__ double gather_load(const double *p) {
#if ABFT_CFG_GATHER == 1
  return __builtin_nontemporal_load(p);
#elif ABFT_CFG_GATHER == 2
  return __hip_atomic_load(p, __ATOMIC_RELAXED, __HIP_MEMORY_SCOPE_AGENT);
#else
  return *p;
// ... 550 lines not shown
    double l1[8], l2[4], l3[2];
#pragma unroll
    for (int e = 0; e < 8; e++) l1[e] = (idx & 1u) ? pal[2 * e + 1] : pal[2 * e];
#pragma unroll
    for (int e = 0; e < 4; e++) l2[e] = (idx & 2u) ? l1[2 * e + 1] : l1[2 * e];
#pragma unroll
    for (int e = 0; e < 2; e++) l3[e] = (idx & 4u) ? l2[2 * e + 1] : l2[2 * e];
    val[j] = (idx & 8u) ? l3[1] : l3[0];
#else
    val[j] = cp.pal[pbase + idx];
#endif
    ok[j] = i >= lo && i < hi;
  }
  double xv[EPT];
#pragma unroll
  for (int j = 0; j < EPT; j++) {
    const bool in = ok[j] && col[j] < A.n_in;
    xv[j] = gather_load(x + (in ? col[j] : 0u));
    if (!in) xv[j] = 0.0;
  }
  uint32_t xbad = 0u;
  if (VECC) xbad = vecc_decode_gathers<EPT>(xv);
#pragma unroll
  for (int s = 0; s < STEPS; s++) {
    const uint32_t k = 2u * threadIdx.x + (uint32_t)s * (2u * ABFT_BLOCK);
    const double p0 = val[2 * s] * xv[2 * s], p1 = val[2 * s + 1] * xv[2 * s + 1];
    *reinterpret_cast<double2 *>(s_prod + k) = make_double2(ok[2 * s] ? p0 : 0.0, ok[2 * s + 1] ? p1 : 0.0);
  }
  if (VECC && __builtin_expect(xbad != 0u, 0)) vecc_redo_gathers<EPT>(xbad, x, col, val, ev, s_prod);
}

__device__ __forceinline__ bool csr_check_element(const CsrDev &A, const EventRing &ev, uint32_t base, uint32_t i,
                                                  uint32_t re, uint32_t row_end, const uint32_t *s_col,
                                                  uint32_t row) {
  const uint32_t k = i - base;
  const uint32_t col = s_col[k];
  if (col >= A.n_in) {
    push_event(ev, ABFT_EV_COL_SIZE, A.index_base + i, row, FMT_CSR);
    return false;
  }
  if (i + 1u < row_end) {
    const uint32_t nxt = (i + 1u < re) ? s_col[k + 1u] : A.cols[i + 1u];
    if (nxt <= col) {
      push_event(ev, ABFT_EV_COL_ORDER, A.index_base + i, row, FMT_CSR);
      return false;
    }
  }
  return true;
}

template <int MODE, bool SHORT = false>
__device__ __forceinline__ bool csr_row_sum(const CsrDev &A, const EventRing &ev, uint32_t base,
                                            uint32_t rs, uint32_t re, uint32_t row_end,
                                            const double *s_prod, const uint32_t *s_col,
                                            double &acc, uint32_t row = 0) {
  if (MODE != MODE_CONSTRAINTS && SHORT) {
    for (uint32_t i = rs; i < re; i += 2u) {
      const uint32_t k = i - base, last = re - 1u - base;
      const double a0 = s_prod[k], a1 = s_prod[min(k + 1u, last)];
      acc += a0;
      if (i + 1u < re) acc += a1;
    }
    return true;
  }
  if (MODE != MODE_CONSTRAINTS) {
    for (uint32_t i = rs; i < re; i += 4u) {
      const uint32_t k = i - base, last = re - 1u - base;
      const double a0 = s_prod[k], a1 = s_prod[min(k + 1u, last)], a2 = s_prod[min(k + 2u, last)],
                   a3 = s_prod[min(k + 3u, last)];
      acc += a0;
      if (i + 1u < re) acc += a1;
      if (i + 2u < re) acc += a2;
      if (i + 3u < re) acc += a3;
    }
    return true;
  }
  for (uint32_t i = rs; i < re; i++) {
    if (!csr_check_element(A, ev, base, i, re, row_end, s_col, row)) return false;
    acc += s_prod[i - base];
  }
  return true;
}

template <int MODE, int EPT, bool FUSE, bool VECC = false>
__global__ __launch_bounds__(ABFT_BLOCK) void spmv_csr_kernel(CsrDev A, const double *__restrict__ x,
                                                              double *__restrict__ y, EventRing ev,
                                                              FuseOut fuse, TileSpan span, CsrCompact cc,
                                                              CsrPacked cp) {
  constexpr uint32_t TILE = ABFT_BLOCK * EPT;
  __shared__ __attribute__((aligned(16))) double s_prod[TILE];
  __shared__ __attribute__((aligned(16))) uint32_t s_col[MODE == MODE_CONSTRAINTS ? TILE : 2];
  const uint32_t b = xcd_tile(blockIdx.x, span.count);
  const uint32_t t = span.first + b + (b >= span.cut ? span.skip : 0u);
  const uint4 desc = A.blk[t];
  const uint32_t cb = (MODE == MODE_NONE && cc.cbase) ? cc.cbase[t] : ABFT_CBASE_WIDE;
  const uint2 pd = (MODE == MODE_NONE && cp.pdesc) ? cp.pdesc[t] : make_uint2(0u, 0u);
  const bool uniform = ABFT_CFG_UNIFORM_ROWS && MODE != MODE_CONSTRAINTS && (desc.y >> 31) != 0u;
  const uint32_t row0 = desc.x, row1 = desc.y & 0x7fffffffu, e0 = desc.z, e1 = desc.w;
  const uint32_t base = e0 & ~1u;
  double dsum = 0.0;

  if (e1 >= e0 && e1 - base <= TILE) {
    const uint32_t r = row0 + threadIdx.x;
    uint32_t rs = 0, re = 0;
    double xr = 0.0;
    if (r < row1) {
      if (uniform) {
        const uint32_t len = (e1 - e0) / (row1 - row0);
        rs = e0 + len * threadIdx.x; re = rs + len;
      } else {
        rs = A.rowptr[r]; re = A.rowptr[r + 1];
      }
      if (FUSE) xr = x[fuse.x_off + r];
    }
    if (MODE == MODE_NONE && pd.y != 0u)
      csr_stage_packed<EPT, VECC>(A, cp, pd, x, ev, base, e0, e1, s_prod);
    else if (MODE == MODE_NONE)
      csr_stage_none<EPT, VECC>(A, cc, cb, x, ev, base, e0, e1, s_prod, s_col);
    else
      csr_stage<MODE, EPT, VECC>(A, x, ev, base, e0, e1, s_prod, s_col);
    __syncthreads();
    for (uint32_t row = r; row < row1; row += ABFT_BLOCK) {
      if (row != r) {
        rs = A.rowptr[row]; re = A.rowptr[row + 1];
        if (FUSE) xr = x[fuse.x_off + row];
      }
      if (MODE == MODE_CONSTRAINTS) {
        if (re > A.nnz) { push_event(ev, ABFT_EV_ROW_SIZE, row, row, FMT_CSR); continue; }
        if (re < rs) { push_event(ev, ABFT_EV_ROW_ORDER, row, row, FMT_CSR); continue; }
      }
      if (rs < e0 || re > e1 || re < rs) continue;
      double acc = 0.0;
      if (csr_row_sum<MODE>(A, ev, base, rs, re, re, s_prod, s_col, acc, row)) {
        if (VECC) {
          const uint64_t yw = vecc_encode(acc);
          y[row] = vecc_double(yw);
          if (FUSE) {
            uint64_t xw = vecc_bits(xr);
            if (__builtin_expect(vecc_suspect(xw) != 0u, 0)) xw = vecc_cold(xw, fuse.x_off + row, 0u, ev).w;
            dsum += vecc_value(xw) * vecc_value(yw);
          }
        } else {
          y[row] = acc;
          if (FUSE) dsum += xr * acc;
        }
      }
    }
  } else {
    for (uint32_t row = row0; row < row1; row++) {
      const uint32_t rs = A.rowptr[row], re = A.rowptr[row + 1];
      if (MODE == MODE_CONSTRAINTS) {
        if (re > A.nnz) { if (threadIdx.x == 0) push_event(ev, ABFT_EV_ROW_SIZE, row, row, FMT_CSR); continue; }
        if (re < rs) { if (threadIdx.x == 0) push_event(ev, ABFT_EV_ROW_ORDER, row, row, FMT_CSR); continue; }
      }
      if (re > A.nnz || re < rs) continue;
      double acc = 0.0;
      bool ok = true;
      for (uint32_t lo = rs; lo < re;) {
        const uint32_t b = lo & ~1u;
        const uint32_t hi = min(re, b + TILE);
        __syncthreads();
        csr_stage<MODE, EPT, VECC>(A, x, ev, b, lo, hi, s_prod, s_col);
        __syncthreads();
        if (threadIdx.x == 0 && ok) ok = csr_row_sum<MODE>(A, ev, b, lo, hi, re, s_prod, s_col, acc, row);
        lo = hi;
      }
      if (threadIdx.x == 0 && ok) {
        if (VECC) {
          const uint64_t yw = vecc_encode(acc);
          y[row] = vecc_double(yw);
          if (FUSE) dsum += vecc_decode_cold_ok(x + fuse.x_off + row, fuse.x_off + row, 0u, ev) * vecc_value(yw);
        } else {
          y[row] = acc;
          if (FUSE) dsum += x[fuse.x_off + row] * acc;
        }
      }
    }
  }
  if (FUSE) fused_dot_finish(dsum, fuse, t);
}

template <int MODE, int EPT, bool FUSE>
__global__ __launch_bounds__(ABFT_BLOCK) void spmv_csr_panels_kernel(CsrDev A, CsrPanels P,
                                                                     const double *__restrict__ x,
                                                                     double *__restrict__ y, EventRing ev,
                                                                     FuseOut fuse, uint32_t c0, uint32_t c1) {
  constexpr uint32_t TILE = ABFT_BLOCK * EPT;
  constexpr int RPT = ABFT_PANEL_ROWS_PER_THREAD;
  __shared__ __attribute__((aligned(16))) double s_prod[TILE];
  __shared__ __attribute__((aligned(16))) uint32_t s_col[2];
  double dsum = 0.0;
  for (uint32_t g = blockIdx.x; g < P.ngroups; g += gridDim.x) {
    const uint32_t row0 = g * ABFT_PANEL_ROWS;
    double acc[RPT];
#pragma unroll
    for (int j = 0; j < RPT; j++) {
      const uint32_t row = row0 + (uint32_t)j * ABFT_BLOCK + threadIdx.x;
      acc[j] = (c0 > 0 && row < A.n_out) ? y[row] : 0.0;
    }
    for (uint32_t c = c0; c < c1; c++) {
      const uint32_t seg = g * P.npanels + c;
      const uint32_t e0 = P.seg_base[seg], e1 = P.seg_base[seg + 1];
      if (e0 == e1) continue;
      const uint16_t *ptr = P.seg_ptr + (size_t)seg * (ABFT_PANEL_ROWS + 1);
      uint32_t rs[RPT], re[RPT];
#pragma unroll
      for (int j = 0; j < RPT; j++) {
        const uint32_t r = (uint32_t)j * ABFT_BLOCK + threadIdx.x;
        rs[j] = e0 + ptr[r];
        re[j] = e0 + ptr[r + 1];
      }
      for (uint32_t lo = e0; lo < e1;) {
        const uint32_t b = lo & ~1u;
        const uint32_t hi = min(e1, b + TILE);
        __syncthreads();
        csr_stage<MODE, EPT>(A, x, ev, b, lo, hi, s_prod, s_col);
        __syncthreads();
#pragma unroll
        for (int j = 0; j < RPT; j++) {
          const uint32_t a0 = max(rs[j], lo), a1 = min(re[j], hi);
          if (a0 < a1) {
            double t = acc[j];
            csr_row_sum<MODE>(A, ev, b, a0, a1, a1, s_prod, s_col, t);
            acc[j] = t;
          }
        }
        lo = hi;
      }
    }
    double xo[FUSE ? RPT : 1];
    if (FUSE) {
#pragma unroll
      for (int j = 0; j < RPT; j++) xo[j] = x[fuse.x_off + min(row0 + (uint32_t)j * ABFT_BLOCK + threadIdx.x, A.n_out - 1u)];
    }
#pragma unroll
    for (int j = 0; j < RPT; j++) {
      const uint32_t row = row0 + (uint32_t)j * ABFT_BLOCK + threadIdx.x;
      if (row < A.n_out) {
        y[row] = acc[j];
        if (FUSE) dsum += xo[j] * acc[j];
      }
    }
  }
  if (FUSE) fused_dot_finish(dsum, fuse, blockIdx.x);
}

template <int MODE>
static hipError_t launch_panels_mode(const CsrDev &A, const CsrPanels &P, const double *x, double *y,
                                     EventRing ev, const FuseOut *fuse, uint32_t grid, uint32_t c0, uint32_t c1,
                                     hipStream_t s) {
  if (fuse)
    hipLaunchKernelGGL((spmv_csr_panels_kernel<MODE, ABFT_CFG_PANEL_EPT, true>), dim3(grid), dim3(ABFT_BLOCK), 0,
                       s, A, P, x, y, ev, *fuse, c0, c1);
  else
    hipLaunchKernelGGL((spmv_csr_panels_kernel<MODE, ABFT_CFG_PANEL_EPT, false>), dim3(grid), dim3(ABFT_BLOCK), 0,
                       s, A, P, x, y, ev, FuseOut{}, c0, c1);
  return hipGetLastError();
}

hipError_t launch_spmv_csr_panels(int mode, const CsrDev &A, const CsrPanels &P, const double *x, double *y,
                                  EventRing ev, const FuseOut *fuse, uint32_t grid, uint32_t chunk,
                                  hipStream_t s) {
  if (P.ngroups == 0) return hipSuccess;
  if (chunk == 0 || chunk > P.npanels) chunk = P.npanels;
  for (uint32_t c0 = 0; c0 < P.npanels; c0 += chunk) {
    const uint32_t c1 = c0 + chunk < P.npanels ? c0 + chunk : P.npanels;
    const FuseOut *f = c1 == P.npanels ? fuse : nullptr;
    hipError_t e;
    switch (mode) {
      case MODE_NONE: e = launch_panels_mode<MODE_NONE>(A, P, x, y, ev, f, grid, c0, c1, s); break;
      case MODE_SED: e = launch_panels_mode<MODE_SED>(A, P, x, y, ev, f, grid, c0, c1, s); break;
      case MODE_SEC7: e = launch_panels_mode<MODE_SEC7>(A, P, x, y, ev, f, grid, c0, c1, s); break;
      case MODE_SEC8: e = launch_panels_mode<MODE_SEC8>(A, P, x, y, ev, f, grid, c0, c1, s); break;
      case MODE_SECDED: e = launch_panels_mode<MODE_SECDED>(A, P, x, y, ev, f, grid, c0, c1, s); break;
      default: return hipErrorInvalidValue;
    }
    if (e != hipSuccess) return e;
  }
  return hipSuccess;
}

template <int MODE, bool FUSE> static int panels_occupancy() {
  int n = 0;
  if (hipOccupancyMaxActiveBlocksPerMultiprocessor(&n, spmv_csr_panels_kernel<MODE, ABFT_CFG_PANEL_EPT, FUSE>,
                                                   ABFT_BLOCK, 0) != hipSuccess || n < 1)
    n = 1;
  return n > 8 ? 8 : n;
}

int spmv_csr_panels_blocks_per_cu(int mode, bool fuse) {
  switch (mode) {
    case MODE_NONE: return fuse ? panels_occupancy<MODE_NONE, true>() : panels_occupancy<MODE_NONE, false>();
    case MODE_SED: return fuse ? panels_occupancy<MODE_SED, true>() : panels_occupancy<MODE_SED, false>();
    case MODE_SEC7: return fuse ? panels_occupancy<MODE_SEC7, true>() : panels_occupancy<MODE_SEC7, false>();
    case MODE_SEC8: return fuse ? panels_occupancy<MODE_SEC8, true>() : panels_occupancy<MODE_SEC8, false>();
    default: return fuse ? panels_occupancy<MODE_SECDED, true>() : panels_occupancy<MODE_SECDED, false>();
  }
}

template <int MODE>
static hipError_t launch_spmv_csr_mode(const CsrDev &A, const CsrCompact &cc, const CsrPacked &cp, const TileSpan &span,
                                       const double *x, double *y, EventRing ev, const FuseOut *fuse, hipStream_t s,
                                       bool vecc) {
  if (vecc && fuse)
    hipLaunchKernelGGL((spmv_csr_kernel<MODE, ABFT_CSR_EPT, true, true>), dim3(span.count), dim3(ABFT_BLOCK), 0, s, A,
                       x, y, ev, *fuse, span, cc, cp);
  else if (vecc)
    hipLaunchKernelGGL((spmv_csr_kernel<MODE, ABFT_CSR_EPT, false, true>), dim3(span.count), dim3(ABFT_BLOCK), 0, s, A,
                       x, y, ev, FuseOut{}, span, cc, cp);
  else if (fuse) {
    hipLaunchKernelGGL((spmv_csr_kernel<MODE, ABFT_CSR_EPT, true>), dim3(span.count), dim3(ABFT_BLOCK), 0, s, A,
                       x, y, ev, *fuse, span, cc, cp);
  } else
    hipLaunchKernelGGL((spmv_csr_kernel<MODE, ABFT_CSR_EPT, false>), dim3(span.count), dim3(ABFT_BLOCK), 0, s, A,
                       x, y, ev, FuseOut{}, span, cc, cp);
  return hipGetLastError();
}

hipError_t launch_spmv_csr(int mode, const CsrDev &A, const CsrCompact &cc, const CsrPacked &cp, const TileSpan &span,
                           const double *x, double *y, EventRing ev, const FuseOut *fuse, hipStream_t s, bool vecc) {
  if (span.count == 0) return hipSuccess;
  if ((uint64_t)span.first + span.count + span.skip > A.nblk || span.cut > span.count) return hipErrorInvalidValue;
  if ((cc.cbase || cc.cols16) && (mode != MODE_NONE || !cc.cbase || !cc.cols16)) return hipErrorInvalidValue;
  if ((cp.code16 || cp.pdesc || cp.pal) && (mode != MODE_NONE || !cp.code16 || !cp.pdesc || !cp.pal))
    return hipErrorInvalidValue;
  switch (mode) {
    case MODE_NONE: return launch_spmv_csr_mode<MODE_NONE>(A, cc, cp, span, x, y, ev, fuse, s, vecc);
    case MODE_CONSTRAINTS: return launch_spmv_csr_mode<MODE_CONSTRAINTS>(A, cc, cp, span, x, y, ev, fuse, s, vecc);
    case MODE_SED: return launch_spmv_csr_mode<MODE_SED>(A, cc, cp, span, x, y, ev, fuse, s, vecc);
    case MODE_SEC7: return launch_spmv_csr_mode<MODE_SEC7>(A, cc, cp, span, x, y, ev, fuse, s, vecc);
    case MODE_SEC8: return launch_spmv_csr_mode<MODE_SEC8>(A, cc, cp, span, x, y, ev, fuse, s, vecc);
    case MODE_SECDED: return launch_spmv_csr_mode<MODE_SECDED>(A, cc, cp, span, x, y, ev, fuse, s, vecc);
    default: return hipErrorInvalidValue;
  }
}

#define SPMM_NO_COL 0xffffffffu

template <int MODE, int EPT>
__device__ __forceinline__ void spmm_stage(const CsrDev &A, const EventRing &ev, uint32_t base, uint32_t lo,
                                           uint32_t hi, double *s_val, uint32_t *s_col) {
  constexpr int STEPS = EPT / 2;
  CsrTileRegs<EPT> t;
  csr_issue_loads<EPT>(A, base, hi, t);
  uint32_t col[EPT];
  double val[EPT];
  uint32_t bad = 0u;
#pragma unroll
  for (int j = 0; j < EPT; j++) {
    const int s = j >> 1;
    const uint32_t i = base + 2u * threadIdx.x + (uint32_t)s * (2u * ABFT_BLOCK) + (uint32_t)(j & 1);
    const double d = (j & 1) ? t.v[s].y : t.v[s].x;
    uint32_t w[3] = {(uint32_t)__double2loint(d), (uint32_t)__double2hiint(d), (j & 1) ? t.c[s].y : t.c[s].x};
    const bool valid = i >= lo && i < hi;
    if (MODE >= MODE_SED) {
      if (valid && ecc_suspect<FMT_CSR, MODE>(w) != 0) bad |= 1u << j;
      w[2] &= ABFT_COLMASK;
    }
    col[j] = valid ? w[2] : SPMM_NO_COL;
    val[j] = valid ? as_double(w[0], w[1]) : 0.0;
  }
#pragma unroll
  for (int s = 0; s < STEPS; s++) {
    const uint32_t k = 2u * threadIdx.x + (uint32_t)s * (2u * ABFT_BLOCK);
    *reinterpret_cast<double2 *>(s_val + k) = make_double2(val[2 * s], val[2 * s + 1]);
    *reinterpret_cast<uint2 *>(s_col + k) = make_uint2(col[2 * s], col[2 * s + 1]);
  }
  if (MODE >= MODE_SED && __builtin_expect(bad != 0u, 0)) {
#pragma unroll 1
    for (uint32_t j = 0; j < (uint32_t)EPT; j++) {
      if (!((bad >> j) & 1u)) continue;
      const uint32_t i = base + 2u * threadIdx.x + (j >> 1) * (2u * ABFT_BLOCK) + (j & 1u);
      const double d = A.vals[i];
      EccWords<FMT_CSR> e;
      e.w[0] = (uint32_t)__double2loint(d); e.w[1] = (uint32_t)__double2hiint(d); e.w[2] = A.cols[i]; e.rc = 0;
      e = ecc_cold<FMT_CSR, MODE>(e, event_index(A, i), ev);
      double v = 0.0;
      uint32_t c = SPMM_NO_COL;
      if (e.rc > 0) {
        A.vals[i] = as_double(e.w[0], e.w[1]);
        A.cols[i] = e.w[2];
        v = as_double(e.w[0], e.w[1]);
        c = e.w[2] & ABFT_COLMASK;
      }
      s_val[i - base] = v;
      s_col[i - base] = c;
    }
  }
}

template <int K>
__device__ __forceinline__ void spmm_gather(const double *__restrict__ x, uint32_t c, uint32_t n_in, double *xv) {
  const bool in = c < n_in;
  const double *p = x + (size_t)(in ? c : 0u) * K;
  if (K % 2 == 0) {
#pragma unroll
    for (int j = 0; j < K; j += 2) {
      const double2 v = *reinterpret_cast<const double2 *>(p + j);
      xv[j] = in ? v.x : 0.0;
      xv[j + 1] = in ? v.y : 0.0;
    }
  } else {
#pragma unroll
    for (int j = 0; j < K; j++) xv[j] = in ? p[j] : 0.0;
  }
}

template <int MODE, int K>
__device__ __forceinline__ bool spmm_row_sum(const CsrDev &A, const EventRing &ev, const double *__restrict__ x,
                                             uint32_t base, uint32_t rs, uint32_t re, uint32_t row_end,
                                             const double *s_val, const uint32_t *s_col, double *acc,
                                             uint32_t row) {
  if (MODE == MODE_CONSTRAINTS) {
    for (uint32_t i = rs; i < re; i++) {
      if (!csr_check_element(A, ev, base, i, re, row_end, s_col, row)) return false;
// ... 1912 lines not shown
    double v[4];
#pragma unroll
    for (int k = 0; k < 4; k++) {
      const uint32_t j = i + (uint32_t)k * ABFT_BLOCK;
      v[k] = j < hi ? parts[j] : 0.0;
    }
    acc += (v[0] + v[1]) + (v[2] + v[3]);
  }
  acc = block_sum(acc, s_w);
  reduce_finish(acc, out, s_w);
}

hipError_t launch_fuse_finalize(const FuseOut &f, uint32_t nblk, const ReduceOut &big, const FixArgs *fix,
                                hipStream_t s) {
  FixArgs fx{};
  if (fix) fx = *fix;
  if (nblk <= 8192u || !big.partials) {
    hipLaunchKernelGGL(fuse_finalize_kernel, dim3(1), dim3(1024), 0, s, f, nblk, fx);
    return hipGetLastError();
  }
  uint32_t nb = (nblk + 2047u) / 2048u;
  if (nb > 64u) nb = 64u;
  const uint32_t chunk = (nblk + nb - 1u) / nb;
  hipLaunchKernelGGL(fold_partials_kernel, dim3(nb), dim3(ABFT_BLOCK), 0, s, f.partials, nblk, chunk, big, fx);
  return hipGetLastError();
}

template <int VEC>
__global__ __launch_bounds__(ABFT_BLOCK) void dot_kernel(const double *__restrict__ a,
                                                         const double *__restrict__ b, int n,
                                                         ReduceOut out) {
  __shared__ double s_w[4];
  double acc = 0.0;
  const long stride = (long)gridDim.x * ABFT_BLOCK * VEC;
  for (long i = ((long)blockIdx.x * ABFT_BLOCK + threadIdx.x) * VEC; i < n; i += stride) {
    if (VEC == 2 && i + 1 < n) {
      const double2 av = *reinterpret_cast<const double2 *>(a + i);
      const double2 bv = *reinterpret_cast<const double2 *>(b + i);
      acc += av.x * bv.x;
      acc += av.y * bv.y;
    } else {
      acc += a[i] * b[i];
    }
  }
  acc = block_sum(acc, s_w);
  reduce_finish(acc, out, s_w);
}

template <int VEC>
__global__ __launch_bounds__(ABFT_BLOCK) void calc_xr_kernel(double *__restrict__ x, double *__restrict__ r,
                                                             const double *__restrict__ p,
                                                             const double *__restrict__ w, double alpha,
                                                             const double *num, const double *den, int n,
                                                             ReduceOut out) {
  __shared__ double s_w[4];
  if (num) alpha = *num / *den;
  double acc = 0.0;
  const long stride = (long)gridDim.x * ABFT_BLOCK * VEC;
  for (long i = ((long)blockIdx.x * ABFT_BLOCK + threadIdx.x) * VEC; i < n; i += stride) {
    if (VEC == 2 && i + 1 < n) {
      double2 xv = *reinterpret_cast<double2 *>(x + i);
      double2 rv = *reinterpret_cast<double2 *>(r + i);
      const double2 pv = *reinterpret_cast<const double2 *>(p + i);
      const double2 wv = *reinterpret_cast<const double2 *>(w + i);
      xv.x += alpha * pv.x; xv.y += alpha * pv.y;
      rv.x -= alpha * wv.x; rv.y -= alpha * wv.y;
      *reinterpret_cast<double2 *>(x + i) = xv;
      *reinterpret_cast<double2 *>(r + i) = rv;
      acc += rv.x * rv.x;
      acc += rv.y * rv.y;
    } else {
      const double xs = x[i] + alpha * p[i];
      const double rs = r[i] - alpha * w[i];
      x[i] = xs;
      r[i] = rs;
      acc += rs * rs;
    }
  }
  acc = block_sum(acc, s_w);
  reduce_finish(acc, out, s_w);
}

template <int VEC>
__global__ __launch_bounds__(ABFT_BLOCK) void calc_p_kernel(double *__restrict__ p, const double *__restrict__ r,
                                                            double beta, const double *num, const double *den,
                                                            int n) {
  if (num) beta = *num / *den;
  const long stride = (long)gridDim.x * ABFT_BLOCK * VEC;
  for (long i = ((long)blockIdx.x * ABFT_BLOCK + threadIdx.x) * VEC; i < n; i += stride) {
    if (VEC == 2 && i + 1 < n) {
      double2 pv = *reinterpret_cast<double2 *>(p + i);
      const double2 rv = *reinterpret_cast<const double2 *>(r + i);
      pv.x = rv.x + beta * pv.x;
      pv.y = rv.y + beta * pv.y;
      *reinterpret_cast<double2 *>(p + i) = pv;
    } else {
      p[i] = r[i] + beta * p[i];
    }
  }
}

static inline bool aligned16(const void *a, const void *b = nullptr, const void *c = nullptr,
                             const void *d = nullptr) {
  return (((uintptr_t)a | (uintptr_t)b | (uintptr_t)c | (uintptr_t)d) & 15u) == 0;
}

hipError_t launch_dot(const double *a, const double *b, int n, const ReduceOut &out, hipStream_t s) {
  const int nb = reduce_blocks(n);
  if (aligned16(a, b))
    hipLaunchKernelGGL(dot_kernel<2>, dim3(nb), dim3(ABFT_BLOCK), 0, s, a, b, n, out);
  else
    hipLaunchKernelGGL(dot_kernel<1>, dim3(nb), dim3(ABFT_BLOCK), 0, s, a, b, n, out);
  return hipGetLastError();
}

hipError_t launch_calc_xr(double *x, double *r, const double *p, const double *w, double alpha,
                          const double *num, const double *den, int n, const ReduceOut &out, hipStream_t s) {
  const int nb = reduce_blocks(n);
  if (aligned16(x, r, p, w))
    hipLaunchKernelGGL(calc_xr_kernel<2>, dim3(nb), dim3(ABFT_BLOCK), 0, s, x, r, p, w, alpha, num, den, n, out);
  else
    hipLaunchKernelGGL(calc_xr_kernel<1>, dim3(nb), dim3(ABFT_BLOCK), 0, s, x, r, p, w, alpha, num, den, n, out);
  return hipGetLastError();
}

hipError_t launch_calc_p(double *p, const double *r, double beta, const double *num, const double *den, int n,
                         hipStream_t s) {
  if (n <= 0) return hipSuccess;
  const int nb = reduce_blocks(n);
  if (aligned16(p, r))
    hipLaunchKernelGGL(calc_p_kernel<2>, dim3(nb), dim3(ABFT_BLOCK), 0, s, p, r, beta, num, den, n);
  else
    hipLaunchKernelGGL(calc_p_kernel<1>, dim3(nb), dim3(ABFT_BLOCK), 0, s, p, r, beta, num, den, n);
  return hipGetLastError();
}


template <int VEC>
__global__ __launch_bounds__(ABFT_BLOCK) void calc_r_kernel(const double *r, const double *__restrict__ w,
                                                            double alpha, const double *num, const double *den,
                                                            double *alpha_out, int n, ReduceOut out, double *r_out) {
  __shared__ double s_w[4];
  if (num) alpha = *num / *den;
  if (alpha_out && blockIdx.x == 0 && threadIdx.x == 0) *alpha_out = alpha;
  double acc = 0.0;
  const long stride = (long)gridDim.x * ABFT_BLOCK * VEC;
  for (long i = ((long)blockIdx.x * ABFT_BLOCK + threadIdx.x) * VEC; i < n; i += stride) {
    if (VEC == 2 && i + 1 < n) {
      double2 rv = *reinterpret_cast<const double2 *>(r + i);
#if ABFT_CFG_DEAD_NT & 1
      typedef double v2d __attribute__((ext_vector_type(2)));
      const v2d wl = __builtin_nontemporal_load(reinterpret_cast<const v2d *>(w + i));
      const double2 wv = make_double2(wl.x, wl.y);
#else
      const double2 wv = *reinterpret_cast<const double2 *>(w + i);
#endif
      rv.x -= alpha * wv.x; rv.y -= alpha * wv.y;
      *reinterpret_cast<double2 *>(r_out + i) = rv;
      acc += rv.x * rv.x;
      acc += rv.y * rv.y;
    } else {
      const double rs = r[i] - alpha * w[i];
      r_out[i] = rs;
      acc += rs * rs;
    }
  }
  acc = block_sum(acc, s_w);
  reduce_finish(acc, out, s_w);
}

template <int VEC>
__global__ __launch_bounds__(ABFT_BLOCK) void calc_px_kernel(const double *p, const double *__restrict__ r,
                                                             const double *x, double beta,
                                                             const double *num, const double *den, double alpha,
                                                             const double *alpha_ptr, int n, double *p_out, double *x_out) {
  if (num) beta = *num / *den;
  if (alpha_ptr) alpha = *alpha_ptr;
  const long stride = (long)gridDim.x * ABFT_BLOCK * VEC;
  for (long i = ((long)blockIdx.x * ABFT_BLOCK + threadIdx.x) * VEC; i < n; i += stride) {
    if (VEC == 2 && i + 1 < n) {
#if ABFT_CFG_X_NT || (ABFT_CFG_DEAD_NT & 6) || ABFT_CFG_PX_OUT_NT
      typedef double v2d __attribute__((ext_vector_type(2)));
#endif
#if ABFT_CFG_DEAD_NT & 4
      const v2d pl = __builtin_nontemporal_load(reinterpret_cast<const v2d *>(p + i));
      double2 pv = make_double2(pl.x, pl.y);
#else
      double2 pv = *reinterpret_cast<const double2 *>(p + i);
#endif
#if ABFT_CFG_X_NT
      const v2d xl = __builtin_nontemporal_load(reinterpret_cast<const v2d *>(x + i));
      double2 xv = make_double2(xl.x, xl.y);
#else
      double2 xv = *reinterpret_cast<const double2 *>(x + i);
#endif
#if ABFT_CFG_DEAD_NT & 2
      const v2d rl = __builtin_nontemporal_load(reinterpret_cast<const v2d *>(r + i));
      const double2 rv = make_double2(rl.x, rl.y);
#else
      const double2 rv = *reinterpret_cast<const double2 *>(r + i);
#endif
      xv.x += alpha * pv.x; xv.y += alpha * pv.y;
      pv.x = rv.x + beta * pv.x;
      pv.y = rv.y + beta * pv.y;
#if ABFT_CFG_X_NT
      __builtin_nontemporal_store(v2d{xv.x, xv.y}, reinterpret_cast<v2d *>(x_out + i));
#elif ABFT_CFG_PX_OUT_NT & 1
      if (x_out != x) __builtin_nontemporal_store(v2d{xv.x, xv.y}, reinterpret_cast<v2d *>(x_out + i));
      else *reinterpret_cast<double2 *>(x_out + i) = xv;
#else
      *reinterpret_cast<double2 *>(x_out + i) = xv;
#endif
#if ABFT_CFG_PX_OUT_NT & 2
      if (p_out != p) __builtin_nontemporal_store(v2d{pv.x, pv.y}, reinterpret_cast<v2d *>(p_out + i));
      else *reinterpret_cast<double2 *>(p_out + i) = pv;
#else
// ... 1878 lines not shown
```

include/abft_hip.h:

```cpp
#ifndef ABFT_HIP_H
#define ABFT_HIP_H

#include <stddef.h>
#include <stdint.h>

#ifdef __cplusplus
extern "C" {
#endif

#define ABFT_OK 0
#define ABFT_ERR_INVALID (-1)
#define ABFT_ERR_HIP (-2)
#define ABFT_ERR_NOMEM (-3)
#define ABFT_ERR_RANGE (-4)
#define ABFT_ERR_NODEVICE (-5)

typedef enum {
  ABFT_MODE_NONE = 0,
  ABFT_MODE_CONSTRAINTS = 1,
  ABFT_MODE_SED = 2,
  ABFT_MODE_SEC7 = 3,
  ABFT_MODE_SEC8 = 4,
  ABFT_MODE_SECDED = 5
} abft_mode;
// ... 163 lines not shown
                           uint32_t active);
int abft_hip_calc_r_precond_block(abft_hip_ctx *ctx, abft_hip_vector *R, const abft_hip_vector *W,
                                  const abft_hip_vector *dinv, int k, const double *alpha, uint32_t active,
                                  double *out);
int abft_hip_calc_px_precond_block(abft_hip_ctx *ctx, abft_hip_vector *X, abft_hip_vector *P,
                                   const abft_hip_vector *R, const abft_hip_vector *dinv, int k,
                                   const double *alpha, const double *beta, uint32_t active);

int abft_hip_dot_dev(abft_hip_ctx *ctx, const abft_hip_vector *a, const abft_hip_vector *b,
                     double *dev_result);
int abft_hip_calc_xr_dev(abft_hip_ctx *ctx, abft_hip_vector *x, abft_hip_vector *r,
                         const abft_hip_vector *p, const abft_hip_vector *w, double alpha,
                         double *dev_result);
int abft_hip_read_pair(abft_hip_ctx *ctx, const double *dev_pair, double *value, double *events);
int abft_hip_write_pair(abft_hip_ctx *ctx, double *dev_pair, double value, double events);

size_t abft_hip_peer_board_bytes(void);
int abft_hip_peer_board_attach(abft_hip_ctx *ctx, void *shared, size_t bytes, int rank, int size,
                               double timeout_seconds);
int abft_hip_peer_board_detach(abft_hip_ctx *ctx);
int abft_hip_allreduce_pair_peers(abft_hip_ctx *ctx, double *dev_pair);
int abft_hip_peer_board_fuse(abft_hip_ctx *ctx, int on);
int abft_hip_peer_board_failed(abft_hip_ctx *ctx);
size_t abft_hip_peer_board_ipc_handle_bytes(void);
int abft_hip_peer_board_ipc_export(abft_hip_ctx *ctx, void *handle);
int abft_hip_peer_board_ipc_attach(abft_hip_ctx *ctx, const void *handles, int rank, int size, double timeout_seconds);
int abft_hip_peer_board_device_alloc(abft_hip_ctx *ctx, void **board);
int abft_hip_peer_board_device_free(abft_hip_ctx *ctx, void *board);
int abft_hip_peer_board_attach_device(abft_hip_ctx *ctx, void *const *boards, int rank, int size, double timeout_seconds);

typedef struct {
  int peer;
  uint32_t vector_offset;
  uint32_t count;
  uint64_t box_offset;
} abft_peer_piece;
size_t abft_hip_peer_exchange_bytes(int size, size_t outbox_bytes);
int abft_hip_peer_exchange_attach(abft_hip_ctx *ctx, void *shared, size_t bytes, int rank, int size,
                                  size_t outbox_bytes, const abft_peer_piece *out, int nout,
                                  const abft_peer_piece *in, int nin, double timeout_seconds);
int abft_hip_peer_exchange_detach(abft_hip_ctx *ctx);
int abft_hip_peer_exchange(abft_hip_ctx *ctx, abft_hip_vector *full);
int abft_hip_peer_exchange_begin(abft_hip_ctx *ctx, abft_hip_vector *full, int beside);
int abft_hip_peer_exchange_finish(abft_hip_ctx *ctx);
int abft_hip_peer_exchange_failed(abft_hip_ctx *ctx);
int abft_hip_peer_exchange_ipc_export(abft_hip_ctx *ctx, int size, size_t outbox_bytes, void *handle);
int abft_hip_peer_exchange_ipc_attach(abft_hip_ctx *ctx, const void *handles, int rank, int size, size_t outbox_bytes,
                                      const abft_peer_piece *out, int nout, const abft_peer_piece *in, int nin,
                                      double timeout_seconds);
int abft_hip_peer_exchange_device_alloc(abft_hip_ctx *ctx, int size, size_t outbox_bytes, void **region);
int abft_hip_peer_exchange_device_free(abft_hip_ctx *ctx, void *region);
int abft_hip_peer_exchange_attach_device(abft_hip_ctx *ctx, void *const *regions, int rank, int size, size_t outbox_bytes,
                                         const abft_peer_piece *out, int nout, const abft_peer_piece *in, int nin,
                                         double timeout_seconds);

int abft_hip_spmv_dot_dev(abft_hip_ctx *ctx, abft_hip_matrix *mat, const abft_hip_vector *vec,
                          abft_hip_vector *result, int vec_offset, double *dev_result);
int abft_hip_calc_xr_ratio_dev(abft_hip_ctx *ctx, abft_hip_vector *x, abft_hip_vector *r,
                               const abft_hip_vector *p, const abft_hip_vector *w,
                               const double *dev_num, const double *dev_den, double *dev_result);
int abft_hip_calc_p_ratio_dev(abft_hip_ctx *ctx, abft_hip_vector *p, const abft_hip_vector *r,
                              const double *dev_num, const double *dev_den);

typedef enum { ABFT_PART_ALL = 0, ABFT_PART_INTERIOR = 1, ABFT_PART_BOUNDARY = 2 } abft_part;
int abft_hip_matrix_set_interior(abft_hip_matrix *mat, int row_lo, int row_hi);
int abft_hip_spmv_part(abft_hip_ctx *ctx, abft_hip_matrix *mat, const abft_hip_vector *vec,
                       abft_hip_vector *result, int part);
int abft_hip_spmv_dot_part_dev(abft_hip_ctx *ctx, abft_hip_matrix *mat, const abft_hip_vector *vec,
                               abft_hip_vector *result, int vec_offset, double *dev_result, int part);

int abft_hip_matrix_panels(abft_hip_matrix *mat, int *npanels, int *width);
int abft_hip_spmv_dot_range_dev(abft_hip_ctx *ctx, abft_hip_matrix *mat, const abft_hip_vector *vec,
                                abft_hip_vector *result, int vec_offset, double *dev_result, int c0, int c1);

int abft_hip_speculation_stats(abft_hip_ctx *ctx, long *taken, long *dropped);

int abft_hip_set_sharers(abft_hip_ctx *ctx, int processes);

int abft_hip_cg_iteration_dev(abft_hip_ctx *ctx, abft_hip_matrix *mat, const abft_hip_vector *vec, int vec_offset,
                              int part, abft_hip_vector *x, abft_hip_vector *r, abft_hip_vector *p,
                              abft_hip_vector *w, const double *dev_rr, double *dev_pw, double *dev_rr_new);
int abft_hip_tail_stats(abft_hip_ctx *ctx, int *path, int *grid, int *want, long counts[4]);

int abft_hip_cg_iteration_until_dev(abft_hip_ctx *ctx, abft_hip_matrix *mat, const abft_hip_vector *vec,
                                    int vec_offset, int part, abft_hip_vector *x, abft_hip_vector *r,
                                    abft_hip_vector *p, abft_hip_vector *w, const double *dev_rr,
                                    double *dev_pw, double *dev_rr_new, double threshold);


typedef struct abft_hip_graph abft_hip_graph;
int abft_hip_graph_begin(abft_hip_ctx *ctx);
int abft_hip_graph_end(abft_hip_ctx *ctx, abft_hip_graph **graph);
int abft_hip_graph_launch(abft_hip_graph *graph);
int abft_hip_graph_destroy(abft_hip_graph *graph);


int abft_hip_drain_events(abft_hip_ctx *ctx, abft_event *buf, int cap, int *count, int *fatal);
int abft_hip_event_capacity(void);
int abft_hip_pending_events(abft_hip_ctx *ctx);
int abft_format_event(const abft_event *ev, char *buf, size_t cap);
int abft_event_is_fatal(uint32_t kind);


typedef enum {
  ABFT_K_SPMV = 0,
  ABFT_K_DOT = 1,
  ABFT_K_CALC_XR = 2,
  ABFT_K_CALC_P = 3,
  ABFT_K_COUNT = 4
} abft_kernel_id;

int abft_hip_profile_enable(abft_hip_ctx *ctx, int mask);
int abft_hip_profile_stride(abft_hip_ctx *ctx, int stride);
int abft_hip_profile_reset(abft_hip_ctx *ctx);
int abft_hip_profile_read(abft_hip_ctx *ctx, int kernel, double *total_ms, long *launches);

int abft_hip_stream_probe(abft_hip_ctx *ctx, size_t bytes, int reps, double *gbps_copy,
                          double *gbps_read);

#ifdef __cplusplus
}
#endif
#endif
```

Before: 4634 CG iterations/s.

## Defer x update into next SpMV via double-buffered p shadow

When the deferred x += alpha*p_old would otherwise be fused into calc_p, calc_p now writes the new p into a shadow buffer and swaps pointers, keeping p_old alive. The pending x update is then folded into the following CSR SpMV kernel, which reads x and p_old per row and writes x. This cuts the traffic calc_p spends touching x and avoids a separate pass. In exchange it allocates an extra vector, adds extra loads and stores inside the bandwidth-bound SpMV, and relies on host-side prediction with a flush fallback when the pattern breaks.

New measurement: 4895 CG iterations/s, median of 6. 1.06x the previous value.

```diff
diff --git a/abft_sparse_cg_amd/capi.py b/abft_sparse_cg_amd/capi.py
--- a/abft_sparse_cg_amd/capi.py
+++ b/abft_sparse_cg_amd/capi.py
@@ -115,6 +115,7 @@
     "abft_hip_speculation_stats": (C.c_int, [vp, C.POINTER(C.c_long), C.POINTER(C.c_long)]),
     "abft_hip_cg_iteration_dev": (C.c_int, [vp, vp, vp, C.c_int, C.c_int, vp, vp, vp, vp, vp, vp, vp]),
     "abft_hip_tail_stats": (C.c_int, [vp, i32p, i32p, i32p, C.POINTER(C.c_long)]),
+    "abft_hip_x_in_spmv_stats": (C.c_int, [vp, C.POINTER(C.c_long), C.POINTER(C.c_long)]),
     "abft_hip_cg_iteration_until_dev": (C.c_int, [vp, vp, vp, C.c_int, C.c_int, vp, vp, vp, vp, vp, vp, vp, C.c_double]),
     "abft_hip_write_pair": (C.c_int, [vp, vp, C.c_double, C.c_double]),
     "abft_hip_peer_board_bytes": (C.c_size_t, []),
diff --git a/abft_sparse_cg_amd/context.py b/abft_sparse_cg_amd/context.py
--- a/abft_sparse_cg_amd/context.py
+++ b/abft_sparse_cg_amd/context.py
@@ -457,6 +457,11 @@
         counts = (C.c_long * 4)()
         check(self.L.abft_hip_tail_stats(self.h, C.byref(path), C.byref(grid), C.byref(want), counts))
         return path.value, grid.value, want.value, list(counts)
+
+    def x_in_spmv_stats(self):
+        absorbed, flushed = C.c_long(0), C.c_long(0)
+        check(self.L.abft_hip_x_in_spmv_stats(self.h, C.byref(absorbed), C.byref(flushed)))
+        return absorbed.value, flushed.value
 
     def cg_iteration_until_dev(self, mat, vec, x, r, p, w, scalars, rr_at, pw_at, rr_new_at, threshold, vec_offset=0,
                                part=capi.PART_ALL):
diff --git a/abft_sparse_cg_amd/csrc/abft_hip.hip b/abft_sparse_cg_amd/csrc/abft_hip.hip
--- a/abft_sparse_cg_amd/csrc/abft_hip.hip
+++ b/abft_sparse_cg_amd/csrc/abft_hip.hip
@@ -96,6 +96,21 @@
     double alpha = 0.0;
   } defer;
   double *alpha_dev = nullptr;
+  bool xin_enabled = true;
+  unsigned xin_modes = ABFT_X_IN_SPMV_MODES;
+  struct {
+    bool armed = false, active = false;
+    const abft_hip_vector *last_p = nullptr;
+    const abft_hip_vector *prev_p = nullptr;
+    double *x = nullptr;
+    const double *p_old = nullptr;
+    double alpha = 0.0;
+    int n = 0;
+    const abft_hip_vector *ph = nullptr;
+    struct { double *buf = nullptr; int n = 0; } shadow[2];
+    int shadow_at = 0;
+    long absorbed = 0, flushed = 0;
+  } xpend;
   double *bpartials = nullptr;
   HostSlotK *bslot = nullptr, *bslot_dev = nullptr;
   HostSlotW *wslot = nullptr, *wslot_dev = nullptr;
@@ -182,6 +197,16 @@
 static_assert(sizeof(abft_event) % sizeof(unsigned long long) == 0, "the table behind the events is 8-byte aligned");
 static constexpr uint32_t MOVED_CAP = 4096;
 
+static int flush_xpend(abft_hip_ctx *ctx) {
+  auto &X = ctx->xpend;
+  if (!X.active) return ABFT_OK;
+  X.active = false;
+  X.armed = false;
+  X.flushed++;
+  HIPCHK(launch_axpy(X.x, X.p_old, X.alpha, nullptr, X.n, ctx->stream));
+  return ABFT_OK;
+}
+
 static int flush_deferred(abft_hip_ctx *ctx) {
   if (!ctx->defer.active) return ABFT_OK;
   ctx->defer.active = false;
@@ -208,10 +233,14 @@
   ctx->spec.x = ctx->spec.r = ctx->spec.p = ctx->spec.w = nullptr;
 }
 
-static int bind(abft_hip_ctx *ctx, bool keep_deferred = false, bool keep_spec = false) {
+static int bind(abft_hip_ctx *ctx, bool keep_deferred = false, bool keep_spec = false, bool keep_xpend = false) {
   if (!ctx) return set_err(ABFT_ERR_INVALID, "null context");
   HIPCHK(hipSetDevice(ctx->device));
+  ctx->xpend.prev_p = ctx->xpend.last_p;
+  ctx->xpend.last_p = nullptr;
   if (!keep_spec) spec_drop(ctx);
+  if (!keep_deferred && !keep_xpend)
+    if (int rc = flush_xpend(ctx)) return rc;
   if (!keep_deferred) return flush_deferred(ctx);
   return ABFT_OK;
 }
@@ -345,6 +374,11 @@
   HIPCHK(hipMalloc((void **)&ctx->spec.scal, 8 * sizeof(double)));
   HIPCHK(hipMemset(ctx->spec.scal, 0, 8 * sizeof(double)));
   if (const char *e = getenv("ABFT_HIP_SPECULATE")) ctx->spec.enabled = strcmp(e, "0") != 0;
+  if (const char *e = getenv("ABFT_HIP_X_IN_SPMV")) {
+    ctx->xin_enabled = strcmp(e, "0") != 0;
+    if (ctx->xin_enabled) ctx->xin_modes = ~0u;
+  }
+  ctx->xin_enabled = ctx->xin_enabled && ctx->defer_enabled && ctx->fuse_enabled && !ctx->spec.enabled;
   HIPCHK(hipHostGetDevicePointer((void **)&ctx->host_slot_dev, ctx->host_slot, 0));
   HIPCHK(hipMalloc((void **)&ctx->ring.buf, EVENT_CAP * sizeof(abft_event) + VECC_SEEN_BYTES));
   HIPCHK(hipMalloc((void **)&ctx->ring.count, sizeof(uint32_t)));
@@ -375,6 +409,7 @@
 extern "C" int abft_hip_shutdown(abft_hip_ctx *ctx) {
   if (!ctx) return ABFT_OK;
   (void)hipSetDevice(ctx->device);
+  (void)flush_xpend(ctx);
   (void)flush_deferred(ctx);
   (void)hipStreamSynchronize(ctx->stream);
   if (debug_leak('d')) (void)hipDeviceSynchronize();
@@ -399,6 +434,7 @@
   if (getenv("ABFT_HIP_VERBOSE") && (ctx->spec.commits || ctx->spec.drops))
     fprintf(stderr, "hip: speculated iterations: %ld taken over, %ld dropped\n", ctx->spec.commits, ctx->spec.drops);
   for (double *b : ctx->spec.shadow) (void)hipFree(b);
+  for (auto &b : ctx->xpend.shadow) (void)hipFree(b.buf);
   (void)hipFree(ctx->spec.scal);
   if (!debug_leak('h')) (void)hipHostFree(ctx->host_slot);
   (void)hipFree(ctx->ring.buf);
@@ -1785,8 +1821,45 @@
   return ABFT_OK;
 }
 
+static bool spec_plain(const abft_hip_vector *v, int n);
+
+static bool xpend_take(abft_hip_ctx *ctx, abft_hip_vector *p, const abft_hip_vector *r, double beta, int *rc) {
+  auto &X = ctx->xpend;
+  *rc = ABFT_OK;
+  if (!ctx->xin_enabled || !X.armed || X.active || ctx->defer.on_dev || ctx->capturing) return false;
+  if (!spec_plain(p, p->n) || !disjoint(p, r)) return false;
+  int at = X.shadow[0].buf && X.shadow[0].n == p->n ? 0 : X.shadow[1].buf && X.shadow[1].n == p->n ? 1 : -1;
+  if (at < 0) {
+    at = X.shadow[X.shadow_at].buf ? 1 - X.shadow_at : X.shadow_at;
+    (void)hipFree(X.shadow[at].buf);
+    X.shadow[at].buf = nullptr;
+    X.shadow[at].n = 0;
+    if (hipMalloc((void **)&X.shadow[at].buf, ((size_t)p->n + 2) * sizeof(double)) != hipSuccess) {
+      (void)hipGetLastError();
+      X.shadow[at].buf = nullptr;
+      ctx->xin_enabled = false;
+      return false;
+    }
+    X.shadow[at].n = p->n;
+  }
+  X.shadow_at = at;
+  {
+    KernelTimer t(ctx, ABFT_K_CALC_P);
+    const hipError_t e = launch_calc_p(p->d, r->d, beta, nullptr, nullptr, p->n, ctx->stream, X.shadow[at].buf);
+    if (e != hipSuccess) {
+      *rc = set_err(ABFT_ERR_HIP, "calc_p: %s", hipGetErrorString(e));
+      return true;
+    }
+  }
+  std::swap(p->d, X.shadow[at].buf);
+  X.active = true;
+  X.x = ctx->defer.x; X.p_old = X.shadow[at].buf; X.alpha = ctx->defer.alpha; X.n = p->n; X.ph = p;
+  return true;
+}
+
 static int calc_p_launch(abft_hip_ctx *ctx, abft_hip_vector *p, const abft_hip_vector *r, double beta,
                          const double *num, const double *den) {
+  if (int rc = flush_xpend(ctx)) return rc;
   if (int rc = check_same(p, r, "calc_p")) return rc;
   ctx->fused.valid = false;
   if (ctx->defer.active) {
@@ -1794,6 +1867,13 @@
     xv.d = ctx->defer.x; xv.n = ctx->defer.n;
     if (ctx->defer.p == p->d && ctx->defer.n == p->n && disjoint(&xv, r)) {
       ctx->defer.active = false;
+      if (!num) {
+        int rc = ABFT_OK;
+        const bool taken = xpend_take(ctx, p, r, beta, &rc);
+        if (rc) return rc;
+        ctx->xpend.last_p = p;
+        if (taken) return ABFT_OK;
+      }
       KernelTimer t(ctx, ABFT_K_CALC_P);
       HIPCHK(launch_calc_px(p->d, r->d, ctx->defer.x, beta, num, den, ctx->defer.alpha,
                             ctx->defer.on_dev ? ctx->alpha_dev : nullptr, p->n, ctx->stream));
@@ -2416,10 +2496,37 @@
   FixArgs fix{};
 };
 
+static bool xpend_predicted(abft_hip_ctx *ctx, const abft_hip_matrix *mat, const abft_hip_vector *vec,
+                            const abft_hip_vector *result, const double *dev_pair, int part, int c1, bool held,
+                            bool vecc) {
+  auto &X = ctx->xpend;
+  const abft_hip_vector *after_calc_p = X.prev_p;
+  X.prev_p = nullptr;
+  if (!ctx->xin_enabled || !mat || !vec || !result) return false;
+  if (mat->fmt != ABFT_FMT_CSR || mat->use_slice || mat->use_sweep || mat->use_panels) return false;
+  if (!(ctx->xin_modes >> (unsigned)mat->mode & 1u)) return false;
+  if (part != ABFT_PART_ALL || c1 >= 0 || dev_pair || held || vecc || ctx->capturing) return false;
+  const uint32_t n = mat->csr.n_out;
+  if (!mat->fuse_partials || !ctx->fuse_enabled || n == 0 || mat->csr.n_in != n || mat->csr.nblk == 0 ||
+      (uint32_t)vec->n != n || (uint32_t)result->n != n || !disjoint(vec, result))
+    return false;
+  if (!X.active) {
+    if (after_calc_p == vec && spec_plain(vec, vec->n)) X.armed = true;
+    return false;
+  }
+  abft_hip_vector xv, pv;
+  xv.d = X.x; xv.n = X.n;
+  pv.d = const_cast<double *>(X.p_old); pv.n = X.n;
+  return X.ph == vec && (uint32_t)X.n == n && disjoint(&xv, result) && disjoint(&pv, result);
+}
+
 static int spmv_common(abft_hip_ctx *ctx, abft_hip_matrix *mat, const abft_hip_vector *vec,
                        abft_hip_vector *result, int vec_offset, double *dev_pair, int part = ABFT_PART_ALL,
                        int c0 = 0, int c1 = -1, HeldFold *hold = nullptr, bool vecc = false) {
-  if (int rc = bind(ctx)) return rc;
+  if (int rc = bind(ctx, false, false, true)) return rc;
+  const bool absorb = xpend_predicted(ctx, mat, vec, result, dev_pair, part, c1, hold != nullptr, vecc);
+  if (!absorb)
+    if (int rc = flush_xpend(ctx)) return rc;
   if (!mat || !vec || !result) return set_err(ABFT_ERR_INVALID, "spmv: null argument");
   if (vecc) {
     spec_forget(ctx);
@@ -2496,10 +2603,15 @@
       else
         HIPCHK(launch_spmv_coo_panels(mat->mode, mat->coo, mat->panels, vec->d, result->d, ctx->ring,
                                       do_fuse ? &fuse : nullptr, mat->panel_grid, mat->panel_chunk, ctx->stream));
-    } else if (mat->fmt == ABFT_FMT_CSR)
+    } else if (mat->fmt == ABFT_FMT_CSR) {
+      const XUpd xu{ctx->xpend.x, ctx->xpend.p_old, ctx->xpend.alpha};
       HIPCHK(launch_spmv_csr(mat->mode, mat->csr, mat->compact, mat->packed, span, vec->d, result->d, ctx->ring,
-                             do_fuse ? &fuse : nullptr, ctx->stream, vecc));
-    else
+                             do_fuse ? &fuse : nullptr, ctx->stream, vecc, absorb ? &xu : nullptr));
+      if (absorb) {
+        ctx->xpend.active = false;
+        ctx->xpend.absorbed++;
+      }
+    } else
       HIPCHK(launch_spmv_coo(mat->mode, mat->coo, vec->d, result->d, ctx->ring, do_fuse ? &fuse : nullptr, ctx->stream));
     if (mat->fmt == ABFT_FMT_COO) {
       fix = make_fix_args(mat->mode, mat->coo, mat->use_panels ? &mat->panels : nullptr, vec->d, result->d,
@@ -3027,6 +3139,7 @@
                                        const abft_hip_vector *dinv, double beta) {
   if (int rc = check_precond("calc_p_precond", {r}, {p}, dinv)) return rc;
   if (int rc = bind_precond(ctx, true)) return rc;
+  if (int rc = flush_xpend(ctx)) return rc;
   if (ctx->defer.active) {
     abft_hip_vector xv;
     xv.d = ctx->defer.x; xv.n = ctx->defer.n;
@@ -3422,6 +3535,13 @@
   return ABFT_OK;
 }
 
+extern "C" int abft_hip_x_in_spmv_stats(abft_hip_ctx *ctx, long *absorbed, long *flushed) {
+  if (!ctx) return set_err(ABFT_ERR_INVALID, "null context");
+  if (absorbed) *absorbed = ctx->xpend.absorbed;
+  if (flushed) *flushed = ctx->xpend.flushed;
+  return ABFT_OK;
+}
+
 
 struct abft_hip_graph {
   abft_hip_ctx *ctx = nullptr;
@@ -3432,6 +3552,7 @@
 extern "C" int abft_hip_graph_begin(abft_hip_ctx *ctx) {
   if (int rc = bind(ctx)) return rc;
   if (ctx->prof) return set_err(ABFT_ERR_INVALID, "graph capture with kernel brackets enabled (abft_hip_profile_enable)");
+  ctx->xin_enabled = false;
   HIPCHK(hipStreamBeginCapture(ctx->stream, hipStreamCaptureModeThreadLocal));
   ctx->capturing = true;
   return ABFT_OK;
diff --git a/abft_sparse_cg_amd/csrc/abft_internal.h b/abft_sparse_cg_amd/csrc/abft_internal.h
--- a/abft_sparse_cg_amd/csrc/abft_internal.h
+++ b/abft_sparse_cg_amd/csrc/abft_internal.h
@@ -130,6 +130,15 @@
 #ifndef ABFT_CFG_PX_OUT_NT
 #define ABFT_CFG_PX_OUT_NT 0
 #endif
+#ifndef ABFT_X_IN_SPMV_MODES
+#define ABFT_X_IN_SPMV_MODES 0x01u
+#endif
+#ifndef ABFT_CFG_XUPD_NT
+#define ABFT_CFG_XUPD_NT 7
+#endif
+#ifndef ABFT_CFG_P_OUT_NT
+#define ABFT_CFG_P_OUT_NT 1
+#endif
 #ifndef ABFT_CFG_X_NT
 #define ABFT_CFG_X_NT 0
 #endif
@@ -231,6 +240,12 @@
 
 struct TileSpan {
   uint32_t first, cut, skip, count;
+};
+
+struct XUpd {
+  double *xs;
+  const double *p_old;
+  double alpha;
 };
 
 hipError_t launch_spmv_sweep(int mode, int rpt, const CsrDev &A, const SweepLayout &L, const double *x, double *y,
@@ -251,7 +266,7 @@
 hipError_t launch_fuse_finalize(const FuseOut &f, uint32_t nblk, const ReduceOut &big, const FixArgs *fix, hipStream_t s);
 hipError_t launch_spmv_csr(int mode, const CsrDev &A, const CsrCompact &cc, const CsrPacked &cp, const TileSpan &span,
                            const double *x, double *y, EventRing ev, const FuseOut *fuse, hipStream_t s,
-                           bool vecc = false);
+                           bool vecc = false, const XUpd *xu = nullptr);
 hipError_t launch_spmv_coo(int mode, const CooDev &A, const double *x, double *y, EventRing ev,
                            const FuseOut *fuse, hipStream_t s);
 struct FixLayout {
@@ -300,7 +315,7 @@
 hipError_t launch_calc_xr(double *x, double *r, const double *p, const double *w, double alpha,
                           const double *num, const double *den, int n, const ReduceOut &out, hipStream_t s);
 hipError_t launch_calc_p(double *p, const double *r, double beta, const double *num, const double *den, int n,
-                         hipStream_t s);
+                         hipStream_t s, double *p_out = nullptr);
 hipError_t launch_calc_r(double *r, const double *w, double alpha, const double *num, const double *den,
                          double *alpha_out, int n, const ReduceOut &out, hipStream_t s, double *r_out = nullptr,
                          const double *x = nullptr, const double *p = nullptr);
diff --git a/abft_sparse_cg_amd/csrc/kernels.hip b/abft_sparse_cg_amd/csrc/kernels.hip
--- a/abft_sparse_cg_amd/csrc/kernels.hip
+++ b/abft_sparse_cg_amd/csrc/kernels.hip
@@ -656,11 +656,20 @@
   return true;
 }
 
-template <int MODE, int EPT, bool FUSE, bool VECC = false>
+#if ABFT_CFG_XUPD_NT
+#define XUPD_LOAD_P(p) ((ABFT_CFG_XUPD_NT & 1) ? __builtin_nontemporal_load(p) : *(p))
+#define XUPD_LOAD_X(p) ((ABFT_CFG_XUPD_NT & 2) ? __builtin_nontemporal_load(p) : *(p))
+#define XUPD_STORE_X(p, v) do { if (ABFT_CFG_XUPD_NT & 4) __builtin_nontemporal_store((v), (p)); else *(p) = (v); } while (0)
+#else
+#define XUPD_LOAD_P(p) (*(p))
+#define XUPD_LOAD_X(p) (*(p))
+#define XUPD_STORE_X(p, v) (*(p) = (v))
+#endif
+template <int MODE, int EPT, bool FUSE, bool VECC = false, bool XUPD = false>
 __global__ __launch_bounds__(ABFT_BLOCK) void spmv_csr_kernel(CsrDev A, const double *__restrict__ x,
                                                               double *__restrict__ y, EventRing ev,
                                                               FuseOut fuse, TileSpan span, CsrCompact cc,
-                                                              CsrPacked cp) {
+                                                              CsrPacked cp, XUpd xu) {
   constexpr uint32_t TILE = ABFT_BLOCK * EPT;
   __shared__ __attribute__((aligned(16))) double s_prod[TILE];
   __shared__ __attribute__((aligned(16))) uint32_t s_col[MODE == MODE_CONSTRAINTS ? TILE : 2];
@@ -687,6 +696,8 @@
       }
       if (FUSE) xr = x[fuse.x_off + r];
     }
+    double xs = 0.0, po = 0.0;
+    if (XUPD && r < row1) { xs = XUPD_LOAD_X(xu.xs + r); po = XUPD_LOAD_P(xu.p_old + r); }
     if (MODE == MODE_NONE && pd.y != 0u)
       csr_stage_packed<EPT, VECC>(A, cp, pd, x, ev, base, e0, e1, s_prod);
     else if (MODE == MODE_NONE)
@@ -698,7 +709,9 @@
       if (row != r) {
         rs = A.rowptr[row]; re = A.rowptr[row + 1];
         if (FUSE) xr = x[fuse.x_off + row];
-      }
+        if (XUPD) { xs = XUPD_LOAD_X(xu.xs + row); po = XUPD_LOAD_P(xu.p_old + row); }
+      }
+      if (XUPD) XUPD_STORE_X(xu.xs + row, xs + xu.alpha * po);
       if (MODE == MODE_CONSTRAINTS) {
         if (re > A.nnz) { push_event(ev, ABFT_EV_ROW_SIZE, row, row, FMT_CSR); continue; }
         if (re < rs) { push_event(ev, ABFT_EV_ROW_ORDER, row, row, FMT_CSR); continue; }
@@ -721,6 +734,8 @@
       }
     }
   } else {
+    if (XUPD)
+      for (uint32_t row = row0 + threadIdx.x; row < row1; row += ABFT_BLOCK) XUPD_STORE_X(xu.xs + row, XUPD_LOAD_X(xu.xs + row) + xu.alpha * XUPD_LOAD_P(xu.p_old + row));
     for (uint32_t row = row0; row < row1; row++) {
       const uint32_t rs = A.rowptr[row], re = A.rowptr[row + 1];
       if (MODE == MODE_CONSTRAINTS) {
@@ -875,36 +890,42 @@
 template <int MODE>
 static hipError_t launch_spmv_csr_mode(const CsrDev &A, const CsrCompact &cc, const CsrPacked &cp, const TileSpan &span,
                                        const double *x, double *y, EventRing ev, const FuseOut *fuse, hipStream_t s,
-                                       bool vecc) {
-  if (vecc && fuse)
+                                       bool vecc, const XUpd *xu) {
+  if (xu)
+    hipLaunchKernelGGL((spmv_csr_kernel<MODE, ABFT_CSR_EPT, true, false, true>), dim3(span.count), dim3(ABFT_BLOCK), 0,
+                       s, A, x, y, ev, *fuse, span, cc, cp, *xu);
+  else if (vecc && fuse)
     hipLaunchKernelGGL((spmv_csr_kernel<MODE, ABFT_CSR_EPT, true, true>), dim3(span.count), dim3(ABFT_BLOCK), 0, s, A,
-                       x, y, ev, *fuse, span, cc, cp);
+                       x, y, ev, *fuse, span, cc, cp, XUpd{});
   else if (vecc)
     hipLaunchKernelGGL((spmv_csr_kernel<MODE, ABFT_CSR_EPT, false, true>), dim3(span.count), dim3(ABFT_BLOCK), 0, s, A,
-                       x, y, ev, FuseOut{}, span, cc, cp);
+                       x, y, ev, FuseOut{}, span, cc, cp, XUpd{});
   else if (fuse) {
     hipLaunchKernelGGL((spmv_csr_kernel<MODE, ABFT_CSR_EPT, true>), dim3(span.count), dim3(ABFT_BLOCK), 0, s, A,
-                       x, y, ev, *fuse, span, cc, cp);
+                       x, y, ev, *fuse, span, cc, cp, XUpd{});
   } else
     hipLaunchKernelGGL((spmv_csr_kernel<MODE, ABFT_CSR_EPT, false>), dim3(span.count), dim3(ABFT_BLOCK), 0, s, A,
-                       x, y, ev, FuseOut{}, span, cc, cp);
+                       x, y, ev, FuseOut{}, span, cc, cp, XUpd{});
   return hipGetLastError();
 }
 
 hipError_t launch_spmv_csr(int mode, const CsrDev &A, const CsrCompact &cc, const CsrPacked &cp, const TileSpan &span,
-                           const double *x, double *y, EventRing ev, const FuseOut *fuse, hipStream_t s, bool vecc) {
+                           const double *x, double *y, EventRing ev, const FuseOut *fuse, hipStream_t s, bool vecc,
+                           const XUpd *xu) {
+  if (xu && (!fuse || vecc || span.first || span.skip || span.count != A.nblk || !span.count || !xu->xs || !xu->p_old))
+    return hipErrorInvalidValue;
   if (span.count == 0) return hipSuccess;
   if ((uint64_t)span.first + span.count + span.skip > A.nblk || span.cut > span.count) return hipErrorInvalidValue;
   if ((cc.cbase || cc.cols16) && (mode != MODE_NONE || !cc.cbase || !cc.cols16)) return hipErrorInvalidValue;
   if ((cp.code16 || cp.pdesc || cp.pal) && (mode != MODE_NONE || !cp.code16 || !cp.pdesc || !cp.pal))
     return hipErrorInvalidValue;
   switch (mode) {
-    case MODE_NONE: return launch_spmv_csr_mode<MODE_NONE>(A, cc, cp, span, x, y, ev, fuse, s, vecc);
-    case MODE_CONSTRAINTS: return launch_spmv_csr_mode<MODE_CONSTRAINTS>(A, cc, cp, span, x, y, ev, fuse, s, vecc);
-    case MODE_SED: return launch_spmv_csr_mode<MODE_SED>(A, cc, cp, span, x, y, ev, fuse, s, vecc);
-    case MODE_SEC7: return launch_spmv_csr_mode<MODE_SEC7>(A, cc, cp, span, x, y, ev, fuse, s, vecc);
-    case MODE_SEC8: return launch_spmv_csr_mode<MODE_SEC8>(A, cc, cp, span, x, y, ev, fuse, s, vecc);
-    case MODE_SECDED: return launch_spmv_csr_mode<MODE_SECDED>(A, cc, cp, span, x, y, ev, fuse, s, vecc);
+    case MODE_NONE: return launch_spmv_csr_mode<MODE_NONE>(A, cc, cp, span, x, y, ev, fuse, s, vecc, xu);
+    case MODE_CONSTRAINTS: return launch_spmv_csr_mode<MODE_CONSTRAINTS>(A, cc, cp, span, x, y, ev, fuse, s, vecc, xu);
+    case MODE_SED: return launch_spmv_csr_mode<MODE_SED>(A, cc, cp, span, x, y, ev, fuse, s, vecc, xu);
+    case MODE_SEC7: return launch_spmv_csr_mode<MODE_SEC7>(A, cc, cp, span, x, y, ev, fuse, s, vecc, xu);
+    case MODE_SEC8: return launch_spmv_csr_mode<MODE_SEC8>(A, cc, cp, span, x, y, ev, fuse, s, vecc, xu);
+    case MODE_SECDED: return launch_spmv_csr_mode<MODE_SECDED>(A, cc, cp, span, x, y, ev, fuse, s, vecc, xu);
     default: return hipErrorInvalidValue;
   }
 }
@@ -2983,20 +3004,26 @@
 }
 
 template <int VEC>
-__global__ __launch_bounds__(ABFT_BLOCK) void calc_p_kernel(double *__restrict__ p, const double *__restrict__ r,
+__global__ __launch_bounds__(ABFT_BLOCK) void calc_p_kernel(const double *p, const double *__restrict__ r,
                                                             double beta, const double *num, const double *den,
-                                                            int n) {
+                                                            int n, double *p_out) {
   if (num) beta = *num / *den;
   const long stride = (long)gridDim.x * ABFT_BLOCK * VEC;
   for (long i = ((long)blockIdx.x * ABFT_BLOCK + threadIdx.x) * VEC; i < n; i += stride) {
     if (VEC == 2 && i + 1 < n) {
-      double2 pv = *reinterpret_cast<double2 *>(p + i);
+      double2 pv = *reinterpret_cast<const double2 *>(p + i);
       const double2 rv = *reinterpret_cast<const double2 *>(r + i);
       pv.x = rv.x + beta * pv.x;
       pv.y = rv.y + beta * pv.y;
-      *reinterpret_cast<double2 *>(p + i) = pv;
+#if ABFT_CFG_P_OUT_NT
+      typedef double v2d __attribute__((ext_vector_type(2)));
+      if (p_out != p) __builtin_nontemporal_store(v2d{pv.x, pv.y}, reinterpret_cast<v2d *>(p_out + i));
+      else *reinterpret_cast<double2 *>(p_out + i) = pv;
+#else
+      *reinterpret_cast<double2 *>(p_out + i) = pv;
+#endif
     } else {
-      p[i] = r[i] + beta * p[i];
+      p_out[i] = r[i] + beta * p[i];
     }
   }
 }
@@ -3026,13 +3053,14 @@
 }
 
 hipError_t launch_calc_p(double *p, const double *r, double beta, const double *num, const double *den, int n,
-                         hipStream_t s) {
+                         hipStream_t s, double *p_out) {
   if (n <= 0) return hipSuccess;
   const int nb = reduce_blocks(n);
-  if (aligned16(p, r))
-    hipLaunchKernelGGL(calc_p_kernel<2>, dim3(nb), dim3(ABFT_BLOCK), 0, s, p, r, beta, num, den, n);
+  if (!p_out) p_out = p;
+  if (aligned16(p, r, p_out))
+    hipLaunchKernelGGL(calc_p_kernel<2>, dim3(nb), dim3(ABFT_BLOCK), 0, s, p, r, beta, num, den, n, p_out);
   else
-    hipLaunchKernelGGL(calc_p_kernel<1>, dim3(nb), dim3(ABFT_BLOCK), 0, s, p, r, beta, num, den, n);
+    hipLaunchKernelGGL(calc_p_kernel<1>, dim3(nb), dim3(ABFT_BLOCK), 0, s, p, r, beta, num, den, n, p_out);
   return hipGetLastError();
 }
 
diff --git a/include/abft_hip.h b/include/abft_hip.h
--- a/include/abft_hip.h
+++ b/include/abft_hip.h
@@ -269,6 +269,8 @@
                               abft_hip_vector *w, const double *dev_rr, double *dev_pw, double *dev_rr_new);
 int abft_hip_tail_stats(abft_hip_ctx *ctx, int *path, int *grid, int *want, long counts[4]);
 
+int abft_hip_x_in_spmv_stats(abft_hip_ctx *ctx, long *absorbed, long *flushed);
+
 int abft_hip_cg_iteration_until_dev(abft_hip_ctx *ctx, abft_hip_matrix *mat, const abft_hip_vector *vec,
                                     int vec_offset, int part, abft_hip_vector *x, abft_hip_vector *r,
                                     abft_hip_vector *p, abft_hip_vector *w, const double *dev_rr,
```
